# mlee03/FRE-NCtools

Measured on AMD Instinct MI355X. Metric: exchange-cells/s, higher is better.
Workload: dtype f64; 1 GPU; C384 cubed sphere (6 tiles) -> 1440x720 lat-lon, conservative_order2: exchange-grid search + centroid pass + CSR build per step; nxgrid=4160000, parallelism=1 latitude band(s) of the target, one per GPU, world_size=1

## Files before the change

### fre-nctools_amd/conserve_interp.py

```python
import ctypes as C
from dataclasses import dataclass, field
from typing import List, Optional

import numpy as np

from . import _lib
from ._lib import lib, check

CONSERVE_ORDER1 = 1
CONSERVE_ORDER2 = 2
TARGET = 16
READ = 256
WRITE = 512
CHECK_CONSERVE = 1024
LEGACY_CLIP = 2048
GREAT_CIRCLE = 4096
MONOTONIC = 16384
CELL_METHODS_MEAN = 0
CELL_METHODS_SUM = 1
MAXVAL = 1.0e20


def _f64(a):
    return np.ascontiguousarray(a, dtype=np.float64)
# ... 41 lines not shown


@dataclass
class FieldConfig:
    data: Optional[np.ndarray] = None
    grad_x: Optional[np.ndarray] = None
    grad_y: Optional[np.ndarray] = None
    grad_mask: Optional[np.ndarray] = None
    area: Optional[np.ndarray] = None
    var: List[VarConfig] = field(default_factory=lambda: [VarConfig()])


def _host_grid_args(grids_in, grid_out, masks):
    nt = len(grids_in)
    keep = []
    dpt = C.POINTER(C.c_double)

    def arr(a, n):
        a = _f64(a).reshape(-1)
        assert a.size == n, (a.size, n)
        keep.append(a)
        return _dp(a)

    def corners(g, a):
        return arr(a, (g.nx + 1) * (g.ny + 1))

    nx = (C.c_int * nt)(*[g.nx for g in grids_in])
    ny = (C.c_int * nt)(*[g.ny for g in grids_in])
    lon = (dpt * nt)(*[corners(g, g.lonc) for g in grids_in])
    lat = (dpt * nt)(*[corners(g, g.latc) for g in grids_in])
    msk = None
    if masks is not None:
        msk = (dpt * nt)(*[arr(m, g.nx * g.ny) if m is not None else dpt() for m, g in zip(masks, grids_in)])
    args = (nt, nx, ny, lon, lat, msk, grid_out.nx, grid_out.ny, corners(grid_out, grid_out.lonc), corners(grid_out, grid_out.latc))
    return args, keep


def _dev_grid_args(nx_in, ny_in, tables_t, masks_t, nx_out, ny_out, out_t, mean_dlat, mean_dlon, device, stream):
    nt = len(nx_in)
    tables = [(C.c_void_p * nt)(*[t.data_ptr() for t in tab]) for tab in tables_t]
    msk = None
    if masks_t is not None:
        msk = (C.c_void_p * nt)(*[(t.data_ptr() if t is not None else None) for t in masks_t])
    use = 0 if stream is None else 1
    sptr = C.c_void_p(0 if stream is None else int(stream))
    return (nt, (C.c_int * nt)(*nx_in), (C.c_int * nt)(*ny_in), *tables, msk, nx_out, ny_out, *[C.c_void_p(t.data_ptr()) for t in out_t],
            float(mean_dlat), float(mean_dlon), device, sptr, use)


class XgridPlan:

    def __init__(self, handle, order, device, great_circle=False):
        self._h = C.c_void_p(handle)
        self.order = order
        self.device = device
        self.great_circle = great_circle

    @classmethod
    def create(cls, order, grids_in, grid_out, masks=None, device=0):
        _lib.require_gpu()
        args, keep = _host_grid_args(grids_in, grid_out, masks)
        h = C.c_void_p()
        check(lib().fg_plan_create(order, *args, device, C.byref(h)))
        return cls(h.value, order, device)

    @classmethod
    def create_dev(cls, order, nx_in, ny_in, lon_in_t, lat_in_t, nx_out, ny_out, lon_out_t, lat_out_t,
                   mean_dlat=0.0, mean_dlon=0.0, device=0, stream=None, masks_t=None):
        h = C.c_void_p()
        check(lib().fg_plan_create_dev(order, *_dev_grid_args(nx_in, ny_in, (lon_in_t, lat_in_t), masks_t, nx_out, ny_out,
                                                              (lon_out_t, lat_out_t), mean_dlat, mean_dlon, device, stream), C.byref(h)))
        return cls(h.value, order, device)

    @classmethod
    def create_great_circle(cls, grids_in, grid_out, masks=None, device=0):
        _lib.require_gpu()
        args, keep = _host_grid_args(grids_in, grid_out, masks)
        h = C.c_void_p()
        check(lib().fg_plan_create_great_circle(*args, device, C.byref(h)))
        return cls(h.value, 1, device, True)

    @classmethod
    def create_great_circle_dev(cls, nx_in, ny_in, xyz_in_t, nx_out, ny_out, xyz_out_t, mean_dlat=0.0, mean_dlon=0.0,
                                device=0, stream=None, masks_t=None):
        h = C.c_void_p()
        tables = [[t[k] for t in xyz_in_t] for k in range(3)]
        check(lib().fg_plan_create_great_circle_dev(*_dev_grid_args(nx_in, ny_in, tables, masks_t, nx_out, ny_out, [xyz_out_t[k] for k in range(3)],
                                                                    mean_dlat, mean_dlon, device, stream), C.byref(h)))
        return cls(h.value, 1, device, True)

    @classmethod
    def create_great_circle_lonlat(cls, grids_in, grid_out, masks=None, device=0):
        _lib.require_gpu()
        args, keep = _host_grid_args(grids_in, grid_out, masks)
        h = C.c_void_p()
        check(lib().fg_plan_create_great_circle_lonlat(*args, device, C.byref(h)))
        return cls(h.value, 1, device, True)

    @classmethod
    def create_great_circle_lonlat_dev(cls, nx_in, ny_in, lon_in_t, lat_in_t, nx_out, ny_out, lon_out_t, lat_out_t,
                                       mean_dlat=0.0, mean_dlon=0.0, device=0, stream=None, masks_t=None):
        h = C.c_void_p()
        check(lib().fg_plan_create_great_circle_lonlat_dev(*_dev_grid_args(nx_in, ny_in, (lon_in_t, lat_in_t), masks_t, nx_out, ny_out,
                                                                           (lon_out_t, lat_out_t), mean_dlat, mean_dlon, device, stream),
                                                           C.byref(h)))
        return cls(h.value, 1, device, True)

    @classmethod
    def create_empty(cls, order, nx_in, ny_in, nx_out, ny_out, device=0):
        _lib.require_gpu()
        nt = len(nx_in)
        h = C.c_void_p()
        check(lib().fg_plan_create_empty(order, nt, (C.c_int * nt)(*nx_in), (C.c_int * nt)(*ny_in),
                                         nx_out, ny_out, device, C.byref(h)))
        return cls(h.value, order, device)

    def destroy(self):
        if self._h is not None and self._h.value:
            lib().fg_plan_destroy(self._h)
        self._h = None

    def __del__(self):
        try:
            self.destroy()
        except Exception:
            pass

    @property
    def nxgrid(self):
        return int(lib().fg_plan_nxgrid(self._h))

    @property
    def ncells_in(self):
        return int(lib().fg_plan_ncells_in(self._h))

    def cell_sums_ptr(self):
        return lib().fg_plan_cell_sums_dev(self._h)

    def copy_cell_sums(self, dst_t):
        check(lib().fg_plan_copy_cell_sums(self._h, C.c_void_p(dst_t.data_ptr())))

    def accumulate_cell_sums(self, total_t, cells_t=None):
        args = (self._h, C.c_void_p(total_t.data_ptr()), C.c_void_p(cells_t.data_ptr()) if cells_t is not None else None,
                int(cells_t.numel()) if cells_t is not None else 0)
        if getattr(total_t, "is_cuda", False):
            cur = _torch().cuda.current_stream(total_t.device)
            if int(self.stream() or 0) == int(cur.cuda_stream):
                check(lib().fg_plan_accumulate_cell_sums_async(*args))
                return
            cur.synchronize()
        check(lib().fg_plan_accumulate_cell_sums(*args))

    def stats(self):
        s = (C.c_long * 10)()
        check(lib().fg_plan_stats(self._h, s, 10))
        names = ["pairs", "nonempty", "nxgrid", "borderline", "bins", "bin_entries", "deferred", "heavy", "below", "exact_mode"]
        return dict(zip(names, [int(v) for v in s]))

    PHASES = ["cell_struct", "bins", "candidates", "clip_quad", "clip_general", "compact", "rows",
              "search_total", "finalize", "apply"]

    def phase_ms(self):
        ms = (C.c_float * 10)()
        check(lib().fg_plan_phase_ms(self._h, ms, 10))
        return dict(zip(self.PHASES, [float(v) for v in ms]))

    def finalize(self, total_sums_ptr=None):
        check(lib().fg_plan_finalize(self._h, C.c_void_p(total_sums_ptr or 0)))

    def sync(self):
        check(lib().fg_plan_sync(self._h))

    def stream(self):
        return lib().fg_plan_stream(self._h)

    def set_stream(self, stream):
        check(lib().fg_plan_set_stream(self._h, C.c_void_p(int(stream))))

    def get_xgrid(self):
        n = self.nxgrid
        ints = {k: np.empty(n, dtype=np.int32) for k in ("t_in", "i_in", "j_in", "i_out", "j_out")}
        area = np.empty(n, dtype=np.float64)
        c1 = np.empty(n, dtype=np.float64) if self.order == 2 else None
        c2 = np.empty(n, dtype=np.float64) if self.order == 2 else None
        check(lib().fg_plan_get_xgrid(self._h, _ip(ints["t_in"]), _ip(ints["i_in"]), _ip(ints["j_in"]),
                                      _ip(ints["i_out"]), _ip(ints["j_out"]), _dp(area), _dp(c1), _dp(c2)))
        out = dict(ints)
        out["area"] = area
        if self.order == 2:
            out["c1"], out["c2"] = c1, c2
        return out

    def get_polygons(self, maxv=16):
        nx = self.nxgrid
        n = np.zeros(nx, dtype=np.int32)
        v = [np.zeros((nx, maxv)) for _ in range(3)]
        check(lib().fg_plan_get_polygons(self._h, maxv, _ip(n), _dp(v[0]), _dp(v[1]), _dp(v[2])))
        if self.great_circle:
            return {"n": n, "x": v[0], "y": v[1], "z": v[2]}
        return {"n": n, "lon": v[0], "lat": v[1]}

    @classmethod
    def create_polylist(cls, order, n, lon, lat, lon_avg, area_ref, grid_out, device=0):
        _lib.require_gpu()
        n = np.ascontiguousarray(n, dtype=np.int32)
        lon, lat = _f64(lon), _f64(lat)
        assert lon.shape == (n.size, 8) == lat.shape
        lon_avg, area_ref = _f64(lon_avg), _f64(area_ref)
        lo, la = _f64(grid_out.lonc).reshape(-1), _f64(grid_out.latc).reshape(-1)
        h = C.c_void_p()
        check(lib().fg_plan_create_polylist(order, n.size, _ip(n), _dp(lon), _dp(lat), _dp(lon_avg), _dp(area_ref), grid_out.nx, grid_out.ny,
                                            _dp(lo), _dp(la), device, C.byref(h)))
        return cls(h.value, order, device)

    def get_cell_area(self, ncells_out):
        a_in = np.empty(self.ncells_in, dtype=np.float64)
        a_out = np.empty(ncells_out, dtype=np.float64)
        check(lib().fg_plan_get_cell_area(self._h, _dp(a_in), _dp(a_out)))
        return a_in, a_out

    def get_cell_struct(self, which, ncells):
        d = {k: np.empty(ncells, dtype=np.float64) for k in ("lat_min", "lat_max", "lon_min", "lon_max", "lon_avg")}
        nv = np.empty(ncells, dtype=np.int32)
        vlon = np.empty((ncells, 8), dtype=np.float64)
        vlat = np.empty((ncells, 8), dtype=np.float64)
        check(lib().fg_plan_get_cell_struct(self._h, which, _dp(d["lat_min"]), _dp(d["lat_max"]), _dp(d["lon_min"]),
                                            _dp(d["lon_max"]), _dp(d["lon_avg"]), _ip(nv), _dp(vlon), _dp(vlat)))
        d.update(nvert=nv, vlon=vlon, vlat=vlat)
        return d

    def set_xgrid(self, t_in, i_in, j_in, i_out, j_out, area, di_in=None, dj_in=None):
        a = [np.ascontiguousarray(v, dtype=np.int32) for v in (t_in, i_in, j_in, i_out, j_out)]
        area = _f64(area)
        di = _f64(di_in) if di_in is not None else None
        dj = _f64(dj_in) if dj_in is not None else None
        check(lib().fg_plan_set_xgrid(self._h, area.size, *[_ip(v) for v in a], _dp(area), _dp(di), _dp(dj)))

    def apply(self, data_t, out_t, nz=1, grad_x_t=None, grad_y_t=None, grad_mask_t=None,
              has_missing=False, missing=-MAXVAL, want_gsum=False):
        g = C.c_double(0.0)
        ptr = lambda t: C.c_void_p(t.data_ptr()) if t is not None else C.c_void_p(0)
        check(lib().fg_plan_apply(self._h, ptr(data_t), ptr(grad_x_t), ptr(grad_y_t), ptr(grad_mask_t),
                                  1 if has_missing else 0, float(missing), nz, ptr(out_t),
                                  C.byref(g) if want_gsum else None))
        return g.value if want_gsum else None


    def apply_ex(self, data_t, out_t, nz=1, grad_x_t=None, grad_y_t=None, grad_mask_t=None, has_missing=False,
                 missing=-MAXVAL, weight_t=None, cell_methods_sum=False, field_area_t=None, area_missing=-MAXVAL,
                 cell_area_in_t=None, cell_area_out_t=None, monotonic=False, want_gsum=False, minmax_hook=None):
        ptr = lambda t: C.c_void_p(t.data_ptr()) if t is not None else C.c_void_p(0)
        addr = lambda t: t.data_ptr() if t is not None else None
        o = _lib.ApplyOpts(1 if has_missing else 0, float(missing), addr(weight_t), 1 if cell_methods_sum else 0,
                           addr(field_area_t), float(area_missing), addr(cell_area_in_t), addr(cell_area_out_t),
                           1 if monotonic else 0)
        g = C.c_double(0.0)
        gp = C.byref(g) if want_gsum else None
        L = lib()
        if monotonic and self.order == 2 and minmax_hook is not None:
            check(L.fg_plan_mono_begin(self._h, C.byref(o), ptr(data_t), ptr(grad_x_t), ptr(grad_y_t), ptr(grad_mask_t)))
            minmax_hook(self)
            check(L.fg_plan_mono_end(self._h, C.byref(o), ptr(data_t), ptr(out_t), gp))
        else:
            check(L.fg_plan_apply_ex(self._h, C.byref(o), ptr(data_t), ptr(grad_x_t), ptr(grad_y_t), ptr(grad_mask_t),
                                     nz, ptr(out_t), gp))
        return g.value if want_gsum else None

    def mono_copy_minmax(self, to_plan, fmin_t, fmax_t):
        check(lib().fg_plan_mono_copy_minmax(self._h, 1 if to_plan else 0, C.c_void_p(fmin_t.data_ptr()),
                                              C.c_void_p(fmax_t.data_ptr())))

    def apply_interleaved(self, nb, data_il_t, out_il_t, grad_x_il_t=None, grad_y_il_t=None, want_gsum=False):
        g = C.c_double(0.0)
        ptr = lambda t: C.c_void_p(t.data_ptr()) if t is not None else C.c_void_p(0)
        check(lib().fg_plan_apply_interleaved(self._h, nb, ptr(data_il_t), ptr(grad_x_il_t), ptr(grad_y_il_t),
                                              ptr(out_il_t), C.byref(g) if want_gsum else None))
        return g.value if want_gsum else None

    def apply_records(self, nz, rec_t, out_t, want_gsum=False):
        g = C.c_double(0.0)
        check(lib().fg_plan_apply_records(self._h, nz, C.c_void_p(rec_t.data_ptr()), C.c_void_p(out_t.data_ptr()),
                                          C.byref(g) if want_gsum else None))
        return g.value if want_gsum else None

    def apply_levels(self, data_t, out_t, nlev, missing, grad_x_t=None, grad_y_t=None, grad_mask_t=None, want_gsum=False):
        g = np.zeros(nlev, dtype=np.float64)
        ptr = lambda t: C.c_void_p(t.data_ptr()) if t is not None else C.c_void_p(0)
        check(lib().fg_plan_apply_levels(self._h, ptr(data_t), ptr(grad_x_t), ptr(grad_y_t), ptr(grad_mask_t), float(missing),
                                         nlev, ptr(out_t), _dp(g) if want_gsum else None))
        return g if want_gsum else None

    def apply_records_levels(self, nz, rec_t, maskbits_t, out_t, missing, want_gsum=False):
        g = np.zeros(nz, dtype=np.float64)
        check(lib().fg_plan_apply_records_levels(self._h, nz, C.c_void_p(rec_t.data_ptr()), C.c_void_p(maskbits_t.data_ptr()),
                                                 float(missing), C.c_void_p(out_t.data_ptr()), _dp(g) if want_gsum else None))
        return g if want_gsum else None

    @staticmethod
    def levels_capacity():
        return int(lib().fg_plan_levels_capacity())


@dataclass
class InterpConfig:
    nxgrid: int = 0
    i_in: Optional[np.ndarray] = None
    j_in: Optional[np.ndarray] = None
    i_out: Optional[np.ndarray] = None
    j_out: Optional[np.ndarray] = None
# ... 248 lines not shown
```

### fre-nctools_amd/csrc/plan.hip

```cpp
#include <hip/hip_runtime.h>
#include <math.h>
#include <stdio.h>
#include <stdlib.h>
#include <string.h>
#include <algorithm>
#include <map>
#include <mutex>
#include <string>
#include <type_traits>
#include <vector>
#include "fg_host.h"
#include "xgrid_device.h"

static thread_local std::string g_err;
extern "C" const char *fg_last_error(void) { return g_err.c_str(); }
void fg_set_last_error(const char *msg) { g_err = msg ? msg : ""; }

extern "C" int fg_device_count(void)
{
  int n = 0;
  hipError_t e = hipGetDeviceCount(&n);
  if (e != hipSuccess) { fg_fail(FG_ERR_HIP, "hipGetDeviceCount: %s", hipGetErrorString(e)); return FG_ERR_HIP; }
  return n;
}
// ... 441 lines not shown
{
  static thread_local FgCounters *h = nullptr;
  if (!h) { if (hipHostMalloc((void **)&h, sizeof(FgCounters), hipHostMallocDefault) != hipSuccess) h = nullptr; }
  return h;
}

struct GcXyz { const double *x, *y, *z; };
struct BoxMode { FgBox box; const double *mask_quad; int no_adjust; };
struct SearchIn {
  const double *const *lon_in = nullptr, *const *lat_in = nullptr, *const *mask_in = nullptr;
  const double *lon_out = nullptr, *lat_out = nullptr;
  const GcXyz *gc_in = nullptr, *gc_out = nullptr;
  const BoxMode *boxm = nullptr;
  double mean_dlat = 0, mean_dlon = 0;
  int rect_hint = 1;
};
struct SearchOpts { bool exact, cull, finalize, rect, dst_frame; int gc_split; bool profile; };
static const char *gc_clip_error(int code)
{
  switch (code) {
    case 3: return "firstIntersect is not in the grid1List";
    case 4: return " not found the next intersection ";
    case 5: return "not return back to the first intersection";
    case 6: return "After clipping, nintersect should be 0";
    case 7: return "inserAfter: point (x,y,z) is not found in the list";
    case 8: return "Error from create_xgrid.c: temp is not in list1";
    default: return "clip_2dx2d_great_circle: more intersections than two convex quadrilaterals can have (list capacity)";
  }
}

static int g_search_cull = 0;
static int g_search_finalize = 0;
static int g_gc_split = 1;
extern "C" void fg_set_gc_split(int on) { g_gc_split = on < 0 ? 0 : on; }
struct SearchCaps { unsigned long long entries; int regcap, nreg; bool rect; };
static int g_search_rect = 1;
extern "C" void fg_set_search_rect(int on) { g_search_rect = on ? 1 : 0; }
static int g_dst_frame = 0;
extern "C" void fg_set_search_frame(int coupler) { g_dst_frame = coupler ? 1 : 0; }
static bool host_says_not_rect(int nx, int ny, const double *lon, const double *lat)
{
  const long nxp = nx + 1;
  const int js[3] = {ny, ny / 2, 1}, is[3] = {nx, nx / 2, 1};
  for (int a = 0; a < 3; a++)
    for (int b = 0; b < 3; b++) {
      const long e = (long)js[a] * nxp + is[b];
      if (memcmp(&lon[e], &lon[is[b]], sizeof(double)) || memcmp(&lat[e], &lat[(long)js[a] * nxp], sizeof(double))) return true;
    }
  return false;
}
#define FG_RETRY (-1000L)
struct Carve {
  size_t n = 0;
  size_t operator()(size_t size) { const size_t at = n; n += size; return at; }
};
struct SearchBlocks {
  fg_plan *pl;
  bool ok = true;
  std::vector<void *> scratch;
  template <typename T> T *keep(size_t count) { T *p = pl->alloc<T>(count); ok = ok && p; return p; }
  template <typename T> T *get(size_t count) { T *p = keep<T>(count); if (p) scratch.push_back(p); return p; }
  void release() { for (void *p : scratch) pl->release(p); scratch.clear(); }
};
static long plan_search_core(fg_plan *pl, const SearchIn &in, const SearchOpts &opt, SearchCaps *caps)
{
  const bool gc = in.gc_in != nullptr;
  const BoxMode *const boxm = in.boxm;
  pl->great_circle = gc;
  hipStream_t st = pl->stream;
  const int nsrc = pl->nsrc, ndst = pl->ndst, order = pl->order;
  FgCounters *hc = pinned_counters();
  if (!hc) return fg_fail(FG_ERR_HIP, "hipHostMalloc failed");

  std::vector<FgTile> &th = pl->tiles_host;
  th.resize(pl->ntiles + 1);
  for (int m = 0; m < pl->ntiles; m++) th[m] = FgTile{gc ? nullptr : in.lon_in[m], gc ? nullptr : in.lat_in[m], pl->nx_in[m], pl->ny_in[m], pl->cell_off[m]};
  th[pl->ntiles] = FgTile{in.lon_out, in.lat_out, pl->nx_out, pl->ny_out, 0};
  pl->tiles_dev = pl->alloc<FgTile>(pl->ntiles + 1);
  if (!pl->tiles_dev) return fg_fail(FG_ERR_HIP, "out of device memory");
  FgTileSet ts; ts.n = 0;
  const bool by_value = !gc && pl->ntiles + 1 <= FG_TILESET_MAX;
  if (by_value) { ts.n = pl->ntiles + 1; for (int m = 0; m <= pl->ntiles; m++) ts.t[m] = th[m]; }
  else FGCHK(hipMemcpyAsync(pl->tiles_dev, th.data(), sizeof(FgTile) * th.size(), hipMemcpyHostToDevice, st));
  FgTileXyz *gct_dev = nullptr;
  std::vector<FgTileXyz> gct;
  if (gc) {
    gct.resize(pl->ntiles + 1);
    for (int m = 0; m < pl->ntiles; m++) gct[m] = FgTileXyz{in.gc_in[m].x, in.gc_in[m].y, in.gc_in[m].z, pl->nx_in[m], pl->ny_in[m], pl->cell_off[m]};
    gct[pl->ntiles] = FgTileXyz{in.gc_out->x, in.gc_out->y, in.gc_out->z, pl->nx_out, pl->ny_out, 0};
    gct_dev = pl->alloc<FgTileXyz>(pl->ntiles + 1);
    if (!gct_dev) return fg_fail(FG_ERR_HIP, "out of device memory");
    FGCHK(hipMemcpyAsync(gct_dev, gct.data(), sizeof(FgTileXyz) * gct.size(), hipMemcpyHostToDevice, st));
  }

  bool any_mask = false;
  if (in.mask_in) for (int m = 0; m < pl->ntiles; m++) if (in.mask_in[m]) any_mask = true;
  if (any_mask) {
    pl->mask_dev = pl->alloc<double>(nsrc);
    if (!pl->mask_dev) return fg_fail(FG_ERR_HIP, "out of device memory");
    std::vector<double> ones;
    for (int m = 0; m < pl->ntiles; m++) {
      size_t nc = (size_t)pl->nx_in[m] * pl->ny_in[m];
      if (in.mask_in[m]) FGCHK(hipMemcpyAsync(pl->mask_dev + pl->cell_off[m], in.mask_in[m], nc * sizeof(double), hipMemcpyDeviceToDevice, st));
      else {
        ones.assign(nc, 1.0);
        FGCHK(hipMemcpyAsync(pl->mask_dev + pl->cell_off[m], ones.data(), nc * sizeof(double), hipMemcpyHostToDevice, st));
        FGCHK(hipStreamSynchronize(st));
      }
    }
  }

  const bool rect = caps->rect && !gc && !boxm;
  pl->rect = rect;
  const double dst_tlon = opt.dst_frame ? (double)NAN : 3.14159265358979323846;
  FgBins bins;
  choose_bins(pl, in.mean_dlat, in.mean_dlon, &bins);
  if (rect) { bins.nblat = 0; bins.nblon = 0; }
  const long nbins = (long)bins.nblat * bins.nblon;
  const long nslots = nbins + bins.nblat;
  const unsigned long long nentries = rect ? 0ull : caps->entries;
  const int ecap = (int)std::min<unsigned long long>(nentries, 2147483647ull);
  FgPairSpace ps{};
  ps.nreg = caps->nreg; ps.regcap = caps->regcap;
  const long npairs = fgd_pairs_total(ps);
  const long nx_alloc = npairs;

  if (!alloc_cells(pl, &pl->S, nsrc)) return fg_fail(FG_ERR_HIP, "out of device memory");
  SearchBlocks blk{pl};
  struct { double *hdr, *lat_ax, *lon_ax, *col, *row, *col_min, *col_max, *col_avg; } rt{};
  if (rect) {
    pl->D = FgCells{};
    pl->D.area = blk.keep<double>(ndst);
    Carve at;
    const size_t o_hdr = at(8), o_lat = at((size_t)pl->ny_out + 1), o_lon = at((size_t)pl->nx_out + 1), o_col = at(8 * (size_t)pl->nx_out),
                 o_row = at(4 * ((size_t)pl->ny_out + 1)), o_cmin = at((size_t)pl->nx_out), o_cmax = at((size_t)pl->nx_out), o_cavg = at((size_t)pl->nx_out);
    double *rect_blk = blk.keep<double>(at.n);
    if (!blk.ok) return fg_fail(FG_ERR_HIP, "out of device memory");
    rt = {rect_blk + o_hdr, rect_blk + o_lat, rect_blk + o_lon, rect_blk + o_col, rect_blk + o_row, rect_blk + o_cmin, rect_blk + o_cmax, rect_blk + o_cavg};
  } else if (!alloc_cells(pl, &pl->D, ndst)) return fg_fail(FG_ERR_HIP, "out of device memory");
  const long t_bins = fgd_scan_tiles(nslots), t_rows = fgd_scan_tiles(ndst), t_comp = fgd_scan_tiles(nsrc);
  const size_t zreg = (size_t)FG_NREG * FG_FILL_STRIDE * sizeof(unsigned);
  Carve z;
  const size_t z_dc = z((sizeof(FgCounters) + 127) / 128 * 128), z_fill = z(zreg), z_tick = z(128);
  const size_t z_lb_bins = z(t_bins * sizeof(unsigned long long)), z_lb_rows = z(t_rows * sizeof(unsigned long long)),
               z_lb_comp = z(t_comp * sizeof(unsigned long long));
  const size_t z_bin_cnt = z((size_t)(nslots + 1) * sizeof(int)), z_bin_fill = z((size_t)(nslots + 1) * sizeof(int)),
               z_row_cnt = z((size_t)(ndst + 1) * sizeof(int)), z_nacc = z((size_t)(nsrc + 1) * sizeof(int));
  z((16 - (z.n - z_bin_cnt) % 16) % 16);
  const size_t z_gc_ntask = z(gc ? zreg : 0), z_gc_ocnt = z(gc ? zreg : 0);
  const size_t zbytes = z.n;
  char *zero_blk = blk.get<char>(zbytes);
  int *bin_start = blk.get<int>(nslots + 1);
  int *heavy_list = blk.get<int>(nsrc + 1);
  int *big_list = blk.get<int>(nsrc + 1);
  int *pair_beg = blk.get<int>(nsrc + 1), *pair_cnt = blk.get<int>(nsrc + 1);
  FgBinEntry *bin_entries = blk.get<FgBinEntry>(nentries ? nentries : 1);
  ps.src = blk.get<int>(npairs + 1); ps.dst = blk.get<int>(npairs + 1);
  double *tmp_area = blk.get<double>(npairs + 1);
  double *tmp_clon = (order == 2) ? blk.get<double>(npairs + 1) : nullptr;
  double *tmp_clat = (order == 2) ? blk.get<double>(npairs + 1) : nullptr;
  int *defer_list = blk.get<int>(npairs + 1);
  const bool early_rows = !gc && !boxm;
  int *tmp_rowpos = early_rows ? blk.get<int>(npairs + 1) : nullptr;
  const bool gc_split = gc && opt.gc_split && npairs < (1L << 28);
  const long tcap_want = (opt.gc_split == 2) ? npairs / 64 : 3 * npairs;
  const long tcap_reg = gc_split ? std::min<long>((tcap_want / FG_NREG + 255) / 256 * 256, 0x7ffffff0L / FG_NREG) : 0;
  const long tcap_all = tcap_reg * FG_NREG;
  unsigned *gc_meta = gc_split ? blk.get<unsigned>(npairs + 1) : nullptr;
  int *gc_tbase = gc_split ? blk.get<int>(npairs + 1) : nullptr;
  int *gc_order = gc_split ? blk.get<int>(npairs + 1) : nullptr;
  unsigned *gc_task = gc_split ? blk.get<unsigned>(tcap_all + 1) : nullptr;
  double *gc_res = gc_split ? blk.get<double>(2 * (size_t)tcap_all + 2) : nullptr;
  pl->xoff = blk.keep<int>(nsrc + 1);
  pl->x_src = blk.keep<int>(nx_alloc + 1); pl->x_dst = blk.keep<int>(nx_alloc + 1);
  pl->x_area = blk.keep<double>(nx_alloc + 1);
  if (order == 2) { pl->x_c1 = blk.keep<double>(nx_alloc + 1); pl->x_c2 = blk.keep<double>(nx_alloc + 1); pl->sums = blk.keep<double>(3 * (size_t)nsrc); }
  int *x_rowpos = blk.get<int>(nx_alloc + 1);
  pl->perm = blk.keep<FgRowEnt>(nx_alloc + 1);
  pl->csr.row_ptr = blk.keep<int>(ndst + 1);
  if (!pl->src_idx_f) pl->src_idx_f = blk.keep<int>(nsrc + 1);
  if (!blk.ok) return fg_fail(FG_ERR_HIP, "out of device memory");
  FgCounters *dc = (FgCounters *)(zero_blk + z_dc);
  ps.fill = (unsigned *)(zero_blk + z_fill);
  unsigned *tickets = (unsigned *)(zero_blk + z_tick);
  unsigned long long *lb_bins = (unsigned long long *)(zero_blk + z_lb_bins), *lb_rows = (unsigned long long *)(zero_blk + z_lb_rows),
                     *lb_comp = (unsigned long long *)(zero_blk + z_lb_comp);
  int *bin_cnt = (int *)(zero_blk + z_bin_cnt), *bin_fill = (int *)(zero_blk + z_bin_fill), *row_cnt = (int *)(zero_blk + z_row_cnt);
  int *nacc = (int *)(zero_blk + z_nacc);
  FGCHK(hipMemsetAsync(zero_blk, 0, zbytes, st));
  if (pl->ll_err) FGCHK(hipMemcpyAsync(&dc->err[2], pl->ll_err, sizeof(unsigned), hipMemcpyDeviceToDevice, st));

  PhaseTimer pt, ptot;
  pt.start(opt.profile, st); ptot.start(opt.profile, st);
  for (int k = 0; k < PH_COUNT; k++) pl->phase_ms[k] = 0;
  ptot.begin(PH_SEARCH_TOTAL);
  pt.begin(PH_CELL_STRUCT);
  if (gc) {
    fgd_gc_cell_struct(gct_dev + pl->ntiles, 1, ndst, pl->D, st, opt.cull ? dc->band_keys : nullptr, 1);
    fgd_gc_cell_struct(gct_dev, pl->ntiles, nsrc, pl->S, st, opt.cull ? dc->band_keys : nullptr, 2);
    fgd_src_field_index(order, pl->tiles_dev, pl->ntiles, nsrc, pl->src_idx_f, st);
  } else if (rect) {
    FgRect &R = pl->rect_tab;
    R.hdr = rt.hdr; R.lat_ax = rt.lat_ax; R.lon_ax = rt.lon_ax; R.col = rt.col; R.row = rt.row;
    R.col_min = rt.col_min; R.col_max = rt.col_max; R.col_avg = rt.col_avg;
    R.bad = &dc->rect_bad; R.nx = pl->nx_out; R.ny = pl->ny_out;
    fgd_rect_tables(in.lon_out, in.lat_out, pl->nx_out, pl->ny_out, rt.hdr, rt.lat_ax, rt.lon_ax, rt.col, rt.col_min, rt.col_max, rt.col_avg, rt.row,
                    &dc->rect_bad, dc->err, st, dst_tlon);
    if (pl->polys.npoly) fgd_polylist_records(pl->polys, pl->S, pl->src_idx_f, pl->sums, &R, heavy_list, &dc->heavy_cnt, dc->err, st);
    fgd_cell_struct2r(ts, pl->tiles_dev, pl->tiles_dev, pl->ntiles, pl->polys.npoly ? 0 : nsrc, ndst, pl->S, pl->D.area, R, pl->mask_dev, order,
                      pl->src_idx_f, pl->sums, dc->err, st, dc->band_keys, (opt.cull && !pl->polys.npoly) ? 2 : 0, heavy_list, &dc->heavy_cnt,
                      ps, pair_beg, pair_cnt, big_list, &dc->big_cnt);
  } else if (opt.cull && !boxm && !pl->polys.npoly) {
    fgd_band_keys(in.lat_out, (long)(pl->nx_out + 1) * (pl->ny_out + 1), dc->band_keys, st);
    fgd_cell_struct2(ts, pl->tiles_dev, pl->tiles_dev, pl->ntiles, nsrc, ndst, pl->S, pl->D, bins, bin_cnt, order, pl->src_idx_f, pl->sums, dc->err, st, dc->band_keys, 2, dst_tlon);
  } else if (pl->polys.npoly) {
    fgd_polylist_records(pl->polys, pl->S, pl->src_idx_f, pl->sums, nullptr, nullptr, nullptr, dc->err, st);
    fgd_cell_struct2(ts, pl->tiles_dev, pl->tiles_dev, pl->ntiles, 0, ndst, pl->S, pl->D, bins, bin_cnt, order, pl->src_idx_f, pl->sums, dc->err, st, nullptr, 0, dst_tlon);
  } else
    fgd_cell_struct2(ts, pl->tiles_dev, pl->tiles_dev, pl->ntiles, nsrc, ndst, pl->S, pl->D, bins, bin_cnt, order, pl->src_idx_f, pl->sums, dc->err, st, nullptr, 0, dst_tlon);
  if (boxm) fgd_box_cell_boxes(boxm->box, pl->S, st);
  if (boxm && boxm->no_adjust) fgd_box_area_no_adjust(boxm->box, pl->S.area, st);
  pt.end();
  pl->have_geom = true;

  if (!rect) {
    pt.begin(PH_BINS);
    if (gc) fgd_bin_count(ndst, pl->D, bins, bin_cnt, st);
    fgd_exclusive_scan1(bin_cnt, nslots, bin_start, lb_bins, &tickets[0], &dc->total[0], dc->err, st);
    fgd_bin_fill(ndst, pl->D, bins, bin_fill, bin_start, bin_entries, ecap, nsrc, pl->S, pl->mask_dev, heavy_list, &dc->heavy_cnt, st);
    pt.end();
  }

  pt.begin(PH_CANDIDATES);
  if (rect)
    fgd_candidates_rect(nsrc, pl->S, pl->mask_dev, pl->rect_tab, ps, pair_beg, pair_cnt, heavy_list, &dc->heavy_cnt, big_list, &dc->big_cnt, st,
                        pl->polys.npoly ? 0 : 1);
  else
    fgd_candidates1(nsrc, pl->S, pl->mask_dev, bins, bin_start, bin_entries, ecap, ps, pair_beg, pair_cnt, heavy_list, &dc->heavy_cnt, big_list,
                    &dc->big_cnt, st);
  pt.end();
  hipEvent_t gc_e1 = nullptr, gc_e2 = nullptr;
  struct EvReturn {
    hipEvent_t &a, &b;
    ~EvReturn() { g_handles.put_sync_event(a); g_handles.put_sync_event(b); a = b = nullptr; }
  } ev_return{gc_e1, gc_e2};
  if (boxm) {
    pt.begin(PH_CLIP_GENERAL);
    fgd_clip_box(order, ps, boxm->box, th[pl->ntiles], pl->S, pl->D, pl->mask_dev, boxm->mask_quad, tmp_area, tmp_clon, tmp_clat, nacc, dc->stats, dc->err, st);
    pt.end();
  } else if (gc) {
    pt.begin(PH_CLIP_GENERAL);
    if (gc_split) {
      if (!pl->stream_b) pl->stream_b = g_handles.get_stream(pl->device);
      gc_e1 = g_handles.get_sync_event(); gc_e2 = g_handles.get_sync_event();
      GcSplit g{gc_meta, gc_tbase, gc_task, gc_res, (unsigned)tcap_reg, (unsigned *)(zero_blk + z_gc_ntask), defer_list, &dc->defer_cnt,
                &dc->gc_list2_cnt, npairs, gc_order, (unsigned *)(zero_blk + z_gc_ocnt)};
      fgd_gc_clip_split(ps, pl->S, pl->mask_dev, pl->D, tmp_area, nacc, g, dc->stats, dc->err, st, pl->stream_b, gc_e1, gc_e2);
    } else
      fgd_gc_clip(ps, pl->S, pl->mask_dev, pl->D, tmp_area, nacc, defer_list, &dc->defer_cnt, dc->stats, dc->err, st);
    pt.end();
  } else {
    pt.begin(PH_CLIP_QUAD);
    fgd_clip_quad(order, ps, pl->S, pl->mask_dev, pl->D, tmp_area, tmp_clon, tmp_clat, nacc, defer_list, &dc->defer_cnt, dc->stats, dc->err, st,
                  rect ? &pl->rect_tab : nullptr, row_cnt, tmp_rowpos);
    pt.end();
    pt.begin(PH_CLIP_GENERAL);
    fgd_clip_general(order, ps, pl->S, pl->mask_dev, pl->D, tmp_area, tmp_clon, tmp_clat, nacc, defer_list, &dc->defer_cnt, dc->stats, dc->err, st,
                     rect ? &pl->rect_tab : nullptr, row_cnt, tmp_rowpos);
    pt.end();
  }
  pt.begin(PH_COMPACT);
  FgCompactIo io{};
  io.pair_beg = pair_beg; io.pair_cnt = pair_cnt;
  io.tmp_area = tmp_area; io.tmp_clon = tmp_clon; io.tmp_clat = tmp_clat;
  io.xoff = pl->xoff; io.x_src = pl->x_src; io.x_dst = pl->x_dst; io.x_area = pl->x_area; io.x_c1 = pl->x_c1; io.x_c2 = pl->x_c2;
  io.row_cnt = row_cnt; io.x_rowpos = x_rowpos; io.sums = pl->sums; io.big_list = big_list; io.big_cnt = &dc->big_cnt;
  io.tmp_rowpos = tmp_rowpos; io.row_ptr = pl->csr.row_ptr; io.perm = pl->perm;
  io.dc = dc; io.xcap = nx_alloc;
  if (early_rows)
    fgd_exclusive_scan2(nacc, nsrc, pl->xoff, lb_comp, &tickets[2], &dc->xtot, row_cnt, ndst, pl->csr.row_ptr, lb_rows, &tickets[1], &dc->rows_total, dc->err, st);
  else
    fgd_exclusive_scan1(nacc, nsrc, pl->xoff, lb_comp, &tickets[2], &dc->xtot, dc->err, st);
  fgd_compact(order, nsrc, ps, io, st);
  pt.end();
  if (!early_rows) {
    pt.begin(PH_ROWS);
    fgd_exclusive_scan1(row_cnt, ndst, pl->csr.row_ptr, lb_rows, &tickets[1], &dc->rows_total, dc->err, st);
    fgd_csr_fill_pos(nx_alloc, &dc->xtot, pl->x_src, pl->x_dst, pl->csr.row_ptr, x_rowpos, pl->perm, st);
    pt.end();
  }
  ptot.end();
  const bool fuse = opt.finalize && early_rows && !pl->polys.npoly;
  int *fused_tmp = nullptr;
  if (fuse) {
    pt.begin(PH_FINALIZE);
    if (order == 2) {
      pl->cen = pl->alloc<FgSrcRec>((size_t)nsrc + 1);
      if (!pl->cen) return fg_fail(FG_ERR_HIP, "out of device memory");
      fgd_centroids(nsrc, pl->S, pl->sums, pl->cen, st);
      pl->csr.e2 = pl->alloc<FgCsrEntry2>(nx_alloc + 1);
    } else pl->csr.e1 = pl->alloc<FgCsrEntry1>(nx_alloc + 1);
    if (!pl->csr.e1 && !pl->csr.e2) return fg_fail(FG_ERR_HIP, "out of device memory");
    int *sg_tmp = pl->alloc<int>(3 * (size_t)(nx_alloc + 1));
    fgd_csr_sortgather(order, ndst, (long)nsrc + ndst, pl->perm, pl->x_area, pl->x_c1, pl->x_c2, pl->src_idx_f,
                       order == 2 ? pl->cen : nullptr, pl->csr, st, sg_tmp, nx_alloc + 1);
    fused_tmp = sg_tmp;
    pt.end();
  }
  FGCHK(hipMemcpyAsync(hc, dc, sizeof(FgCounters), hipMemcpyDeviceToHost, st));
  FGCHK(hipStreamSynchronize(st));
  pt.collect(pl->phase_ms); ptot.collect(pl->phase_ms);
  FGCHK(hipGetLastError());
  if (rect && hc->rect_bad) { caps->rect = false; return FG_RETRY; }
  if (hc->total[0] > nentries) { caps->entries = hc->total[0]; return FG_RETRY; }
  if (hc->total[0] > 2000000000ull) return fg_fail(FG_ERR_ARG, "bin table too large");
  if (hc->total[3] > (unsigned long long)ps.regcap) {
    if (hc->total[3] > 2000000000ull / (unsigned long long)ps.nreg) return fg_fail(FG_ERR_CAPACITY, "candidate pair list exceeds 2^31 entries");
    caps->regcap = (int)((hc->total[3] + FG_REG_ALIGN - 1) / FG_REG_ALIGN * FG_REG_ALIGN);
    return FG_RETRY;
  }
  if (hc->err[2] & G_ERRBIT_LL2X) return fg_fail(FG_ERR_ARG, "latlon2xyz: a grid corner is not finite, or its latitude (|lat| >= 2.4262) or longitude "
                                                          "(|lon| > 1024) lies outside the range of the device trig (radians expected)");
  if (hc->err[0] & 8u) return fg_fail(FG_ERR_ARG, "a grid corner latitude lies outside [-pi/2, pi/2] (radians expected)");
  if (hc->err[0] & 1u) return fg_fail(FG_ERR_MAXV, "create_xgrid.c: n2_in is greater than MAX_V");
  if (hc->err[0] & 2u) return fg_fail(FG_ERR_PARALLEL, "the line between <x1_0,y1_0> and  <x1_1,y1_1> should not parallel to "
                                                    "the line between <x2_0,y2_0> and  <x2_1,y2_1>");
  if (hc->err[0] & 4u) return fg_fail(FG_ERR_MAXV, "clipped polygon exceeds 16 vertices");
  if (hc->err[0] & G_ERRBIT_GC_CONVEX1) return fg_fail(FG_ERR_GEOM, "create_xgrid.c(clip_2dx2d_great_circle): grid box 1 is not convex");
  if (hc->err[0] & G_ERRBIT_GC_CONVEX2) return fg_fail(FG_ERR_GEOM, "create_xgrid.c(clip_2dx2d_great_circle): grid box 2 is not convex");
  if (hc->err[0] & G_ERRBIT_GC_CLIP) return fg_fail(FG_ERR_GEOM, "%s", gc_clip_error((int)hc->err[1]));
  if (hc->err[0] & G_ERRBIT_LOOKBACK) return fg_fail(FG_ERR_HIP, "single-pass scan: a tile waited too long for its predecessor");
  pl->nx = (long)hc->xtot;
  pl->stats[FG_STAT_PAIRS] = (long)hc->total[1];
  pl->stats[FG_STAT_NONEMPTY] = (long)(hc->xtot + hc->stats[FG_STAT_BELOW]);
  pl->stats[FG_STAT_NXGRID] = pl->nx;
  pl->stats[FG_STAT_BORDERLINE] = (long)hc->stats[FG_STAT_BORDERLINE];
  pl->stats[FG_STAT_BINS] = nbins;
  pl->stats[FG_STAT_BIN_ENTRIES] = (long)hc->total[0];
  pl->stats[FG_STAT_DEFERRED] = hc->defer_cnt + hc->gc_list2_cnt;
  pl->stats[FG_STAT_HEAVY] = hc->heavy_cnt;
  pl->stats[FG_STAT_BELOW] = (long)hc->stats[FG_STAT_BELOW];

  pl->rect_tab.bad = nullptr;
  blk.release();
  pl->rows_built = true;
  pl->searched = true;
  if (fuse) {
    pl->release(pl->perm); pl->perm = nullptr; pl->release(fused_tmp);
    if (!pl->red_partial) { pl->red_partial = pl->alloc<double>(1024); pl->red_result = pl->alloc<double>(260); }
    if (!pl->red_partial || !pl->red_result) return fg_fail(FG_ERR_HIP, "out of device memory");
    pl->dist_pending = (order == 2);
    pl->finalized = true; pl->fused = true;
  }
  return pl->nx;
}

static int g_search_exact = 0;
extern "C" void fg_set_search_mode(int exact) { g_search_exact = exact; }
extern "C" void fg_set_search_cull(int on) { g_search_cull = on ? 1 : 0; }
extern "C" void fg_set_search_finalize(int on) { g_search_finalize = on ? 1 : 0; }
static long plan_search(fg_plan *pl, const SearchIn &in)
{
  static const bool env_exact = getenv("FREGRID_HIP_EXACT_SEARCH") && atoi(getenv("FREGRID_HIP_EXACT_SEARCH")) != 0;
  const SearchOpts opt{.exact = g_search_exact || env_exact, .cull = g_search_cull != 0, .finalize = g_search_finalize != 0,
                       .rect = g_search_rect != 0, .dst_frame = g_dst_frame != 0, .gc_split = g_gc_split, .profile = g_profiling != 0};
  const long big = std::max((long)pl->nsrc, (long)pl->ndst);
  if (big > (1L << 28)) return fg_fail(FG_ERR_CAPACITY, "grid of %ld cells: more than 2^28 cells per search are not supported", big);
  SearchCaps caps;
  caps.entries = opt.exact ? 0ull : 3ull * (unsigned long long)pl->ndst + 4096ull;
  const unsigned long long cap_pairs = std::min<unsigned long long>(8ull * (unsigned long long)big + 65536ull, 2000000000ull);
  caps.nreg = (int)std::max(1L, std::min((long)FG_NREG, ((long)pl->nsrc + 1023) / 1024));
  caps.regcap = opt.exact ? 0 : (int)((cap_pairs / caps.nreg + FG_REG_ALIGN - 1) / FG_REG_ALIGN * FG_REG_ALIGN);
  caps.rect = opt.rect && in.rect_hint && !in.gc_in && !in.boxm && pl->nx_out <= 8192 && pl->nx_out >= 2;
  const size_t keep = pl->owned.size();
  long rc = FG_RETRY;
  int attempts = 0;
  for (; attempts < 4 && rc == FG_RETRY; attempts++) {
    if (attempts) {
      (void)hipStreamSynchronize(pl->stream);
      pl->drop_search(keep);
    }
    rc = plan_search_core(pl, in, opt, &caps);
  }
  if (rc == FG_RETRY) return fg_fail(FG_ERR_CAPACITY, "exchange-grid search: capacities did not settle");
  if (rc >= 0) pl->stats[FG_STAT_EXACT] = (attempts > 1) ? 1 : 0;
  return rc;
}

struct CornerSample {
  int nsamp = 0;
  std::vector<double> q;
  const double *corners(int a, int k) const { return &q[((size_t)a * nsamp + k) * 4]; }
};
static long sample_step(int nx, int ny, int *nsamp)
{
  const long ncell = (long)nx * ny;
  long step = ncell / 4096; if (step < 1) step = 1;
  *nsamp = (int)((ncell + step - 1) / step);
  return step;
}
__host__ __device__ static inline void sample_nodes(int nx, long step, int k, long n[4])
{
  const long c = (long)k * step;
  const int i = (int)(c % nx), j = (int)(c / nx);
  n[0] = (long)j * (nx + 1) + i; n[1] = n[0] + 1; n[3] = n[0] + nx + 1; n[2] = n[3] + 1;
}
static CornerSample sample_corners_host(int nx, int ny, int narr, const double *const *arr)
{
  CornerSample s;
  const long step = sample_step(nx, ny, &s.nsamp);
  s.q.resize((size_t)s.nsamp * narr * 4);
  for (int k = 0; k < s.nsamp; k++) {
    long n[4];
    sample_nodes(nx, step, k, n);
    for (int a = 0; a < narr; a++)
      for (int v = 0; v < 4; v++) s.q[((size_t)a * s.nsamp + k) * 4 + v] = arr[a][n[v]];
  }
  return s;
}
__global__ void k_sample_corners(int nx, long step, int nsamp, int narr, const double *a0, const double *a1, const double *a2, double *out)
{
  const int k = blockIdx.x * blockDim.x + threadIdx.x;
  if (k >= nsamp) return;
  long n[4];
  sample_nodes(nx, step, k, n);
  const double *arr[3] = {a0, a1, a2};
  for (int a = 0; a < narr; a++) {
    double *o = out + ((size_t)a * nsamp + k) * 4;
    o[0] = arr[a][n[0]]; o[1] = arr[a][n[1]]; o[2] = arr[a][n[2]]; o[3] = arr[a][n[3]];
  }
}
static int sample_corners_dev(fg_plan *pl, int nx, int ny, int narr, const double *d_a0, const double *d_a1, const double *d_a2, CornerSample *s)
{
  const long step = sample_step(nx, ny, &s->nsamp);
  s->q.resize((size_t)s->nsamp * narr * 4);
  double *d_q = (double *)g_pool.get(pl->device, s->q.size() * sizeof(double));
  if (!d_q) return fg_fail(FG_ERR_HIP, "out of device memory");
  k_sample_corners<<<(s->nsamp + 255) / 256, 256, 0, pl->stream>>>(nx, step, s->nsamp, narr, d_a0, d_a1, d_a2, d_q);
  hipError_t e = hipMemcpyAsync(s->q.data(), d_q, s->q.size() * sizeof(double), hipMemcpyDeviceToHost, pl->stream);
  if (e == hipSuccess) e = hipStreamSynchronize(pl->stream);
  g_pool.put(d_q);
  if (e != hipSuccess) return fg_fail(FG_ERR_HIP, "sampling the destination corners failed: %s", hipGetErrorString(e));
  return 0;
}
static void mean_extents(double sl, double sw, long cnt, double *mdlat, double *mdlon)
{
  const double PI = 3.14159265358979323846;
  if (cnt == 0) { *mdlat = PI / 180; *mdlon = PI / 180; return; }
  *mdlat = sl / cnt; *mdlon = sw / cnt;
  if (*mdlat < 1e-7) *mdlat = 1e-7;
  if (*mdlon < 1e-7) *mdlon = 1e-7;
}
static void extents_lonlat(const CornerSample &s, double *mdlat, double *mdlon, int *curvilinear)
{
  const double PI = 3.14159265358979323846;
  *curvilinear = 0;
  double sl = 0, sw = 0; long cnt = 0;
  for (int k = 0; k < s.nsamp; k++) {
    const double *x = s.corners(0, k), *y = s.corners(1, k);
    if (memcmp(&x[0], &x[3], 8) || memcmp(&x[1], &x[2], 8) || memcmp(&y[0], &y[1], 8) || memcmp(&y[3], &y[2], 8)) *curvilinear = 1;
    double ymin = y[0], ymax = y[0], w = 0;
    for (int m = 1; m < 4; m++) { if (y[m] < ymin) ymin = y[m]; if (y[m] > ymax) ymax = y[m]; }
    for (int m = 0; m < 4; m++) {
      double d = fabs(x[(m + 1) & 3] - x[m]);
      if (d > 3.0 * PI) d = fabs(remainder(d, 2.0 * PI)); else if (d > PI) d = fabs(2.0 * PI - d);
      if (d > w) w = d;
    }
    if (w > PI / 2) continue;
    sl += ymax - ymin; sw += w; cnt++;
  }
  mean_extents(sl, sw, cnt, mdlat, mdlon);
}
static void extents_xyz(const CornerSample &s, double *mdlat, double *mdlon)
{
  double sl = 0, sw = 0; long cnt = 0;
  for (int k = 0; k < s.nsamp; k++) {
    const double *x = s.corners(0, k), *y = s.corners(1, k), *z = s.corners(2, k);
    const double dx = x[0] - x[2], dy = y[0] - y[2], dz = z[0] - z[2];
    const double diag = sqrt(dx * dx + dy * dy + dz * dz);
    const double zc = 0.5 * (z[0] + z[2]);
    const double coslat = sqrt(fmax(0.0, 1.0 - zc * zc));
    if (coslat < 0.2) continue;
    sl += diag; sw += diag / coslat; cnt++;
  }
  mean_extents(sl, sw, cnt, mdlat, mdlon);
}
struct DstExtents { double dlat = 0, dlon = 0; int rect_hint = 1; };
static DstExtents dst_extents_host(int nx, int ny, const double *lon, const double *lat)
{
  const double *arr[2] = {lon, lat};
  DstExtents x;
  int curvilinear;
  extents_lonlat(sample_corners_host(nx, ny, 2, arr), &x.dlat, &x.dlon, &curvilinear);
// ... 1695 lines not shown
```

### fre-nctools_amd/csrc/xgrid_device.h

```cpp
#pragma once
#include <hip/hip_runtime.h>

struct FgTile {
  const double *lon;
  const double *lat;
  int nx, ny;
  int cell_off;
};

struct FgTileXyz {
  const double *x, *y, *z;
  int nx, ny;
  int cell_off;
};
#define G_ERRBIT_GC_CONVEX1 16u
#define G_ERRBIT_GC_CONVEX2 32u
#define G_ERRBIT_GC_CLIP    64u

struct FgCells {
  double *lat_min, *lat_max, *lon_min, *lon_max, *lon_avg, *area;
  int *nv;
  double *verts;
};

struct FgBins {
  int nblat, nblon;
  double inv_wlat, inv_wlon;
};

struct FgBinEntry {
  double lat_min, lat_max, lon_min, lon_max, lon_avg;
  int d;
  int row0;
};

enum {
  FG_STAT_PAIRS = 0,
  FG_STAT_NONEMPTY = 1,
  FG_STAT_NXGRID = 2,
  FG_STAT_BORDERLINE = 3,
  FG_STAT_BINS = 4,
  FG_STAT_BIN_ENTRIES = 5,
  FG_STAT_DEFERRED = 6,
  FG_STAT_HEAVY = 7,
  FG_STAT_BELOW = 8,
  FG_STAT_EXACT = 9,
  FG_NSTATS = 10
};

#define FG_REG_ALIGN 512
#define FG_NREG 64
#define FG_FILL_STRIDE 32
struct FgPairSpace {
  int *src, *dst;
  unsigned *fill;
  int regcap, nreg;
};
#ifdef __HIPCC__
__device__ __forceinline__ bool d_pair_live(const FgPairSpace &ps, int p)
{
  const unsigned first = blockIdx.x * blockDim.x;
  const unsigned r = first / (unsigned)ps.regcap;
  const unsigned f = ps.fill[r * FG_FILL_STRIDE];
  return (unsigned)p - r * (unsigned)ps.regcap < (f < (unsigned)ps.regcap ? f : (unsigned)ps.regcap);
}
#endif
static inline long fgd_pairs_total(const FgPairSpace &ps) { return (long)ps.regcap * ps.nreg; }
#ifdef __HIPCC__
__device__ __forceinline__ unsigned long long d_ord_key(double v)
{
  const unsigned long long b = (unsigned long long)__double_as_longlong(v);
  return (b >> 63) ? ~b : (b | 0x8000000000000000ull);
}
__device__ __forceinline__ double d_ord_val(unsigned long long k)
{
  const unsigned long long b = (k >> 63) ? (k & 0x7fffffffffffffffull) : ~k;
  return __longlong_as_double((long long)b);
}
#endif

#define FG_TILESET_MAX 8
struct FgTileSet { FgTile t[FG_TILESET_MAX]; int n; };

struct FgLl2xGrid { const double *lon, *lat; double *x, *y, *z; long n; };
struct FgLl2xSet { FgLl2xGrid g[FG_TILESET_MAX]; int n; };
#define G_ERRBIT_LL2X 256u
void fgd_latlon2xyz(const FgLl2xGrid *grids, int ngrids, unsigned *err, hipStream_t st);

struct FgCounters {
  unsigned long long total[4];
  unsigned long long rows_total;
  unsigned long long band_keys[2];
  unsigned long long xtot;
  unsigned err[4];
  int heavy_cnt;
  unsigned rect_bad;
  int defer_cnt, big_cnt;
  int gc_list2_cnt;
  unsigned long long stats[FG_NSTATS];
};
#define G_ERRBIT_LOOKBACK 128u

long fgd_scan_tiles(long n);
void fgd_exclusive_scan1(const int *in, long n, int *out, unsigned long long *status, unsigned *ticket,
                         unsigned long long *total_dev, unsigned *err, hipStream_t st);

void fgd_exclusive_scan2(const int *in_a, long n_a, int *out_a, unsigned long long *status_a, unsigned *ticket_a, unsigned long long *total_a,
                         const int *in_b, long n_b, int *out_b, unsigned long long *status_b, unsigned *ticket_b, unsigned long long *total_b,
                         unsigned *err, hipStream_t st);

void fgd_cell_struct2(const FgTileSet &ts, const FgTile *tiles_in, FgTile *tiles_out, int ntiles, int nsrc, int ndst, FgCells S, FgCells D,
                      FgBins b, int *slot_cnt, int order, int *src_idx_f, double *sums, unsigned *err, hipStream_t st,
                      unsigned long long *band_keys = nullptr, int cull = 0, double dst_tlon = 3.14159265358979323846);
void fgd_cell_struct(const FgTile *tiles_dev, int ntiles, int ncells, FgCells c, unsigned *err, hipStream_t st);
void fgd_band_keys(const double *lat, long n, unsigned long long *band_keys, hipStream_t st);
void fgd_bin_count(int ncells, FgCells c, FgBins b, int *slot_cnt, hipStream_t st);
void fgd_bin_fill(int ndst, FgCells D, FgBins b, int *slot_fill, const int *slot_start, FgBinEntry *entries, int cap,
                  int nsrc, FgCells S, const double *mask, int *heavy_list, int *heavy_cnt, hipStream_t st);
void fgd_candidates1(int nsrc, FgCells S, const double *mask, FgBins b, const int *slot_start, const FgBinEntry *entries, int ecap,
                     FgPairSpace ps, int *pair_beg, int *pair_cnt, const int *heavy_list, const int *heavy_cnt, int *big_list, int *big_cnt,
                     hipStream_t st);
#define RECT_COLW 8
struct FgRect {
  const double *lon_ax;
  const double *lat_ax;
  const double *col;
  const double *col_min, *col_max, *col_avg;
  const double *hdr;
  const double *row;
  const unsigned *bad;
  int nx, ny;
};
void fgd_rect_tables(const double *lon, const double *lat, int nx, int ny, double *hdr, double *lat_ax, double *lon_ax, double *col,
                     double *col_min, double *col_max, double *col_avg, double *row, unsigned *bad, unsigned *err, hipStream_t st,
                     double dst_tlon = 3.14159265358979323846);
void fgd_cell_struct2r(const FgTileSet &ts, const FgTile *tiles_in, FgTile *tiles_out, int ntiles, int nsrc, int ndst, FgCells S, double *area_out,
                       FgRect R, const double *mask, int order, int *src_idx_f, double *sums, unsigned *err, hipStream_t st,
                       unsigned long long *band_keys, int cull, int *heavy_list, int *heavy_cnt, FgPairSpace ps, int *pair_beg, int *pair_cnt,
                       int *big_list, int *big_cnt);
void fgd_rect_materialize(int ndst, FgRect R, FgCells D, hipStream_t st);
struct FgPolyList { const int *n; const double *lon, *lat; const double *lon_avg, *area; int npoly; };
void fgd_polylist_records(FgPolyList P, FgCells S, int *src_idx_f, double *sums, const FgRect *rect, int *heavy_list, int *heavy_cnt,
                          unsigned *err, hipStream_t st);
void fgd_candidates_rect(int nsrc, FgCells S, const double *mask, FgRect R, FgPairSpace ps, int *pair_beg, int *pair_cnt,
                         const int *heavy_list, const int *heavy_cnt, int *big_list, int *big_cnt, hipStream_t st, int listed_only);
void fgd_clip_general(int order, FgPairSpace ps, FgCells S, const double *mask, FgCells D,
              double *tmp_area, double *tmp_clon, double *tmp_clat, int *nacc, int *defer_list, int *defer_cnt,
              unsigned long long *stats, unsigned *err, hipStream_t st, const FgRect *rect = nullptr, int *row_cnt = nullptr,
              int *tmp_rowpos = nullptr);
void fgd_clip_quad(int order, FgPairSpace ps, FgCells S, const double *mask, FgCells D,
              double *tmp_area, double *tmp_clon, double *tmp_clat, int *nacc, int *defer_list, int *defer_cnt,
              unsigned long long *stats, unsigned *err, hipStream_t st, const FgRect *rect = nullptr, int *row_cnt = nullptr,
              int *tmp_rowpos = nullptr);
struct alignas(8) FgRowEnt { int n, s; };
struct alignas(16) FgSrcRec { double cen_lon, cen_lat; };
struct FgCompactIo {
  const int *pair_beg, *pair_cnt;
  const double *tmp_area, *tmp_clon, *tmp_clat;
  const int *xoff;
  int *x_src, *x_dst;
  double *x_area, *x_c1, *x_c2;
  int *row_cnt, *x_rowpos;
  const int *tmp_rowpos;
  const int *row_ptr; FgRowEnt *perm;
  double *sums;
  const int *big_list;
  const int *big_cnt;
  FgCounters *dc;
  long xcap;
};
void fgd_compact(int order, int nsrc, FgPairSpace ps, const FgCompactIo &io, hipStream_t st);
void fgd_centroids(int nsrc, FgCells S, const double *sums, FgSrcRec *cen, hipStream_t st);
void fgd_distances(long nx, const int *x_src, const double *x_area, const FgSrcRec *cen, double *x_c1, double *x_c2, hipStream_t st);

struct FgCsrEntry1 { int idx_f; int pad; double area; };
struct FgCsrEntry2 { int idx_f; int idx_g; double area, di, dj; };
struct FgCsr {
  int *row_ptr;
  FgCsrEntry1 *e1;
  FgCsrEntry2 *e2;
};
void fgd_csr_count(long nx, const int *x_dst, int *row_cnt, hipStream_t st);
void fgd_csr_fill(long nx, const int *x_src, const int *x_dst, const int *row_ptr, int *row_fill, FgRowEnt *perm, hipStream_t st);
void fgd_csr_fill_pos(long nx_cap, const unsigned long long *nx_dev, const int *x_src, const int *x_dst, const int *row_ptr, const int *x_rowpos,
                      FgRowEnt *perm, hipStream_t st);
void fgd_csr_sortgather(int order, int ndst, long nx, const FgRowEnt *perm, const double *x_area, const double *x_c1, const double *x_c2,
                        const int *src_idx_f, const FgSrcRec *cen, FgCsr csr, hipStream_t st, int *tmp = nullptr, long ntmp = 0,
                        int long_rows = 0);
void fgd_src_field_index(int order, const FgTile *tiles_dev, int ntiles, int nsrc, int *src_idx_f, hipStream_t st);
void fgd_apply1(int order, int ndst, FgCsr csr, const double *f, const double *gx, const double *gy, const int *gmask,
                int has_missing, double missing, double *out, double *row_sum, hipStream_t st, long nx = -1);
void fgd_apply_il(int order, int nb, int ndst, FgCsr csr, const double *f, const double *gx, const double *gy, double missing,
                  double *out, double *row_sum, long out_ld, int nb_valid, hipStream_t st, long nx = -1);
void fgd_interleave(int nb_pad, long n, const double *in, long ld, int nb_valid, double *out, hipStream_t st);
void fgd_apply_il_merged(int nb, int ndst, long nx, FgCsr csr, const double *rec, double missing, double *out, double *row_sum, long out_ld,
                         int nb_valid, hipStream_t st);
void fgd_merge3(int nb_pad, long n, const int *src_idx_f, const double *f, long ld_f, const double *gx, const double *gy, long ld_g,
                int nb_valid, double *out, hipStream_t st);
void fgd_interleave3(int nb_pad, int narr, const double *const *in, const long *ld, const long *n, double *const *out, int nb_valid,
                     hipStream_t st);
void fgd_deinterleave(int nb_pad, long n, const double *in, long ld, int nb_valid, double *out, hipStream_t st);
#define FG_LEVELS_CAP 256
void fgd_apply_levels8(int order, int ndst, long nx, FgCsr csr, const double *rec, const unsigned char *gbits, double missing, double *out,
                       double *row_sum, long ld, int nb_valid, hipStream_t st);
void fgd_gmask_bits(long n, const int *gmask, long ld, int nb, unsigned char *bits, hipStream_t st);
void fgd_apply_frac(int ndst, FgCsr csr, const double *data, double *out, hipStream_t st);
void fgd_reduce_sum(const double *v, long n, double *partial, double *result, hipStream_t st);
void fgd_xgrid_indices(long nx, const int *x_src, const int *x_dst, const FgTile *tiles_dev, int ntiles, int nx_out,
                       int *t_in, int *i_in, int *j_in, int *i_out, int *j_out, hipStream_t st);

struct FgApplyEx {
  const double *weight;
  const double *cell_area;
  const double *field_area;
  const double *cell_area_out;
  const int *gmask;
  const double *xdata;
  double area_missing, missing;
  int has_missing, sum;
};
#define FG_XERR_AREA_MISSING 1
#define FG_XERR_ABOVE 2
#define FG_XERR_BELOW 4
void fgd_apply_ex(int order, int ndst, FgCsr csr, const double *f, const double *gx, const double *gy, FgApplyEx o,
                  double *out, double *row_sum, int *err, hipStream_t st, long nx = -1);
void fgd_mono_bounds(const FgTile *tiles_dev, int ntiles, int nsrc, const int *src_idx_f, const double *f, double missing,
                     double *fbmax, double *fbmin, double *fmax, double *fmin, hipStream_t st);
void fgd_mono_xdata(long nx, FgCsr csr, const double *f, const double *gx, const double *gy, const int *gmask, double missing,
                    double *xdata, double *fmax, double *fmin, hipStream_t st);
void fgd_mono_limit(long nx, FgCsr csr, const double *f, double missing, const double *fbmax, const double *fbmin,
                    const double *fmax, const double *fmin, double *xdata, int *err, hipStream_t st);

struct FgBox { const double *lon, *lat; int nx, ny; };
void fgd_clip_box(int order, FgPairSpace ps, FgBox box, FgTile quad, FgCells S, FgCells D,
                  const double *mask_box, const double *mask_quad, double *tmp_area, double *tmp_clon, double *tmp_clat, int *nacc,
                  unsigned long long *stats, unsigned *err, hipStream_t st);
void fgd_box_area_no_adjust(FgBox box, double *area, hipStream_t st);
void fgd_box_cell_boxes(FgBox box, FgCells c, hipStream_t st);
void fgd_clip_single(const double *lon_in, const double *lat_in, int n_in, double ll_lon, double ll_lat, double ur_lon, double ur_lat,
                     double *lon_out, double *lat_out, int *n_out, hipStream_t st);
void fgd_box_ctr(double ll_lon, double ll_lat, double ur_lon, double ur_lat, double clon, double *out, hipStream_t st);
void fgd_grid_area_no_adjust(int nx, int ny, const double *lon, const double *lat, double *area, hipStream_t st);

void fgd_accumulate_cell_sums(int n, const int *cells, int nsrc, const int *xoff, const double *xa, const double *c1, const double *c2,
                              double *total, hipStream_t st);

void fgd_gc_cell_struct(const FgTileXyz *tiles_dev, int ntiles, int ncells, FgCells c, hipStream_t st,
                        unsigned long long *band_keys = nullptr, int band_mode = 0);
void fgd_gc_clip(FgPairSpace ps, FgCells S, const double *mask, FgCells D,
                 double *tmp_area, int *nacc, int *defer_list, int *defer_cnt, unsigned long long *stats, unsigned *err, hipStream_t st);
struct GcSplit {
  unsigned *meta;
  int *tbase;
  unsigned *task;
  double *res;
  unsigned tcap;
  unsigned *ntask;
  int *list, *list_cnt;
  int *list2_cnt;
  long list_cap;
  int *order;
  unsigned *ocnt;
};
void fgd_gc_clip_split(FgPairSpace ps, FgCells S, const double *mask, FgCells D, double *tmp_area, int *nacc, GcSplit g,
                       unsigned long long *stats, unsigned *err, hipStream_t st, hipStream_t st2, hipEvent_t e1, hipEvent_t e2);
#define FG_GC_POLY_CAP 16
void fgd_gc_clip_batch(int n, const double *a, const double *b, double *out, int *n_out, double *area, hipStream_t st);
void fgd_gc_area_batch(int npoly, int stride_pts, const double *xyz, const int *n, double *area, hipStream_t st);

#define FG_POLY_STRIDE 24
void fgd_poly_clip(int npoly, const double *lon1, const double *lat1, const int *n1, const double *lon2, const double *lat2,
                   const int *n2, double *lon_out, double *lat_out, int *n_out, hipStream_t st);
void fgd_poly_op(int op, int npoly, double *lon, double *lat, int *n, const double *clon, double *result, hipStream_t st);
void fgd_xgrid_polygons(long n, const int *x_src, const int *x_dst, FgCells S, FgCells D, const FgRect *rect, int maxv,
                        int *n_out, double *lon_out, double *lat_out, hipStream_t st);
void fgd_xgrid_gather_gc(long n, const int *x_src, const int *x_dst, FgCells S, FgCells D, double *a, double *b, hipStream_t st);
void fgd_split_xyz(long n, int maxv, const double *xyz, double *x, double *y, double *z, hipStream_t st);
void fgd_sincos_probe(long n, const double *x, double *s, double *c, hipStream_t st);

void fgd_pack_interior(const void *tiles, int ntiles, long ncells, long F, int nz, const double *src, double *dst, hipStream_t st);
void fgd_halo_gather(long F, int nz, const int *map, double *data, hipStream_t st);
void fgd_grad_c2l(const void *tiles, int ntiles, long ncells, long F, int nz, const double *data, const double *const *geom,
                  double *grad_x, double *grad_y, hipStream_t st);
void fgd_grad_c2l_rec(const void *tiles, int ntiles, long ncells, long F, int nz, int nb_pad, const double *data,
                      const double *const *geom, double *rec, hipStream_t st);
void fgd_c2l_records(const void *tiles, int ntiles, long ncells, int nz, int nb_pad, const double *src, const int *cell_of,
                     const double *const *geom, double *rec, hipStream_t st);
void fgd_c2l_records_levels(const void *tiles, int ntiles, long ncells, int nz, const double *src, const int *cell_of,
                            const double *const *geom, double missing, double *rec, unsigned char *gbits, hipStream_t st);
void fgd_grad_mask(const void *tiles, int ntiles, long ncells, long F, int nz, const double *data, double missing, int *mask, hipStream_t st);
size_t fgd_c2l_tile_size(void);
void fgd_c2l_tile_fill(void *dst, int idx, int nx, int ny, long cell_off, long f_off, long dx_off, long dy_off, long ew_off, long es_off);
```

### fre-nctools_amd/csrc/xgrid_kernels.hip

```cpp
#include <algorithm>
#include "xgrid_device.h"
#ifndef FG_EXP
#define FG_EXP 0
#endif
static __shared__ double fgs_lds_tab[112 * 4];
#define FGS_TAB(k, j) fgs_lds_tab[(k) * 4 + (j)]
#include "geom.hip.h"
__device__ __forceinline__ void d_load_trig_table()
{
  for (int i = threadIdx.x; i < 112 * 4; i += blockDim.x) fgs_lds_tab[i] = FG_SINCOS_TAB[i >> 2][i & 3];
  __syncthreads();
}

#define SCAN_THREADS 256
#define SCAN_ITEMS   8
#define SCAN_CHUNK   (SCAN_THREADS * SCAN_ITEMS)
#define LB_AGG   (1ull << 62)
#define LB_INC   (2ull << 62)
#define LB_MASK  ((1ull << 62) - 1ull)
#define LB_SPIN_LIMIT (1u << 22)

__device__ __forceinline__ unsigned wave_incl_scan(unsigned v, int lane)
{
#pragma unroll
// ... 15 lines not shown
#pragma unroll
  for (int k = 0; k < 4; k++) { if (k < w) base += wsum[k]; tot += wsum[k]; }
  __syncthreads();
  *total = tot;
  return inc + base;
}

__device__ __forceinline__ unsigned long long lb_load(const unsigned long long *p)
{
  return __hip_atomic_load(p, __ATOMIC_RELAXED, __HIP_MEMORY_SCOPE_AGENT);
}
__device__ __forceinline__ void lb_store(unsigned long long *p, unsigned long long v)
{
  __hip_atomic_store(p, v, __ATOMIC_RELAXED, __HIP_MEMORY_SCOPE_AGENT);
}

__device__ inline unsigned long long d_lookback_wave(unsigned long long *status, int tile, unsigned long long agg, unsigned *err)
{
  const int lane = threadIdx.x & 63;
  if (tile == 0) { if (lane == 0) lb_store(&status[0], LB_INC | (agg & LB_MASK)); return 0ull; }
  if (lane == 0) lb_store(&status[tile], LB_AGG | (agg & LB_MASK));
  unsigned long long excl = 0ull;
  int base = tile - 1;
  unsigned spins = 0;
  for (;;) {
    const int t = base - lane;
    const unsigned long long v = (t >= 0) ? lb_load(&status[t]) : LB_INC;
    const unsigned flag = (unsigned)(v >> 62);
    const unsigned long long inc = __ballot(flag == 2u), zero = __ballot(flag == 0u);
    const int first_inc = inc ? (__ffsll((long long)inc) - 1) : 63;
    const unsigned long long need = (first_inc >= 63) ? ~0ull : ((2ull << first_inc) - 1ull);
    if (zero & need) {
      if (++spins > LB_SPIN_LIMIT) { if (lane == 0) atomicOr(err, G_ERRBIT_LOOKBACK); break; }
      __builtin_amdgcn_s_sleep(1);
      continue;
    }
    unsigned long long val = ((need >> lane) & 1ull) ? (v & LB_MASK) : 0ull;
#pragma unroll
    for (int o = 32; o; o >>= 1) val += __shfl_xor(val, o);
    excl += val;
    if (inc) break;
    base -= 64;
  }
  if (lane == 0) lb_store(&status[tile], LB_INC | ((excl + agg) & LB_MASK));
  return excl;
}

__global__ __launch_bounds__(SCAN_THREADS) void k_scan1(const int *in, long n, int *out, unsigned long long *status, unsigned *ticket,
                                                        unsigned long long *total_out, unsigned *err)
{
  __shared__ unsigned tile[SCAN_CHUNK];
  __shared__ int sh_t;
  __shared__ unsigned long long sh_excl;
  if (ticket) { if (threadIdx.x == 0) sh_t = (int)atomicAdd(ticket, 1u); __syncthreads(); }
  const int t = ticket ? sh_t : (int)blockIdx.x;
  const long base = (long)t * SCAN_CHUNK;
#pragma unroll
  for (int k = 0; k < SCAN_ITEMS; k++) {
    const int li = k * SCAN_THREADS + threadIdx.x;
    const long idx = base + li;
    tile[li] = (idx < n) ? (unsigned)in[idx] : 0u;
  }
  __syncthreads();
  unsigned loc[SCAN_ITEMS];
  unsigned s = 0;
#pragma unroll
  for (int k = 0; k < SCAN_ITEMS; k++) { loc[k] = tile[threadIdx.x * SCAN_ITEMS + k]; s += loc[k]; }
  unsigned tot;
  const unsigned inc = block_incl_scan(s, &tot);
  if (threadIdx.x < 64) {
    const unsigned long long e = d_lookback_wave(status, t, (unsigned long long)tot, err);
    if (threadIdx.x == 0) sh_excl = e;
  }
  __syncthreads();
  const unsigned long long excl = sh_excl;
  unsigned run = (unsigned)excl + inc - s;
#pragma unroll
  for (int k = 0; k < SCAN_ITEMS; k++) { tile[threadIdx.x * SCAN_ITEMS + k] = run; run += loc[k]; }
  __syncthreads();
#pragma unroll
  for (int k = 0; k < SCAN_ITEMS; k++) {
    const int li = k * SCAN_THREADS + threadIdx.x;
    const long idx = base + li;
    if (idx <= n) out[idx] = (int)tile[li];
  }
  if (threadIdx.x == 0 && n >= base && n < base + SCAN_CHUNK) *total_out = excl + tot;
}

struct FgScanJob { const int *in; long n; int *out; unsigned long long *status; unsigned *ticket; unsigned long long *total; };
__global__ __launch_bounds__(SCAN_THREADS) void k_scan2(FgScanJob a, FgScanJob b, unsigned *err, int by_ticket)
{
  const FgScanJob j = blockIdx.y ? b : a;
  const long nt = (j.n + 1 + SCAN_CHUNK - 1) / SCAN_CHUNK;
  if ((long)blockIdx.x >= nt) return;
  __shared__ unsigned tile[SCAN_CHUNK];
  __shared__ int sh_t;
  __shared__ unsigned long long sh_excl;
  if (by_ticket) { if (threadIdx.x == 0) sh_t = (int)atomicAdd(j.ticket, 1u); __syncthreads(); }
  const int t = by_ticket ? sh_t : (int)blockIdx.x;
  const long base = (long)t * SCAN_CHUNK;
#pragma unroll
  for (int k = 0; k < SCAN_ITEMS; k++) {
    const int li = k * SCAN_THREADS + threadIdx.x;
    const long idx = base + li;
    tile[li] = (idx < j.n) ? (unsigned)j.in[idx] : 0u;
  }
  __syncthreads();
  unsigned loc[SCAN_ITEMS];
  unsigned s = 0;
#pragma unroll
  for (int k = 0; k < SCAN_ITEMS; k++) { loc[k] = tile[threadIdx.x * SCAN_ITEMS + k]; s += loc[k]; }
  unsigned tot;
  const unsigned inc = block_incl_scan(s, &tot);
  if (threadIdx.x < 64) {
    const unsigned long long e = d_lookback_wave(j.status, t, (unsigned long long)tot, err);
    if (threadIdx.x == 0) sh_excl = e;
  }
  __syncthreads();
  const unsigned long long excl = sh_excl;
  unsigned run = (unsigned)excl + inc - s;
#pragma unroll
  for (int k = 0; k < SCAN_ITEMS; k++) { tile[threadIdx.x * SCAN_ITEMS + k] = run; run += loc[k]; }
  __syncthreads();
#pragma unroll
  for (int k = 0; k < SCAN_ITEMS; k++) {
    const int li = k * SCAN_THREADS + threadIdx.x;
    const long idx = base + li;
    if (idx <= j.n) j.out[idx] = (int)tile[li];
  }
  if (threadIdx.x == 0 && j.n >= base && j.n < base + SCAN_CHUNK) *j.total = excl + tot;
}

long fgd_scan_tiles(long n) { if (n < 0) n = 0; return (n + 1 + SCAN_CHUNK - 1) / SCAN_CHUNK; }
void fgd_exclusive_scan2(const int *in_a, long n_a, int *out_a, unsigned long long *status_a, unsigned *ticket_a, unsigned long long *total_a,
                         const int *in_b, long n_b, int *out_b, unsigned long long *status_b, unsigned *ticket_b, unsigned long long *total_b,
                         unsigned *err, hipStream_t st)
{
  if (n_a < 0) n_a = 0;
  if (n_b < 0) n_b = 0;
  const long nt = std::max(fgd_scan_tiles(n_a), fgd_scan_tiles(n_b));
  k_scan2<<<dim3((unsigned)nt, 2), SCAN_THREADS, 0, st>>>(FgScanJob{in_a, n_a, out_a, status_a, ticket_a, total_a},
                                                         FgScanJob{in_b, n_b, out_b, status_b, ticket_b, total_b}, err, 2 * nt > 1024 ? 1 : 0);
}

void fgd_exclusive_scan1(const int *in, long n, int *out, unsigned long long *status, unsigned *ticket,
                         unsigned long long *total_dev, unsigned *err, hipStream_t st)
{
  if (n < 0) n = 0;
  const int nt = (int)fgd_scan_tiles(n);
  k_scan1<<<nt, SCAN_THREADS, 0, st>>>(in, n, out, status, nt <= 1024 ? nullptr : ticket, total_dev, err);
}


__device__ __forceinline__ int d_cell_record(const FgTile *tiles, int ntiles, int ncells, const FgCells &c, unsigned *err, int s0,
                                             double *vtile, double *box , int *tile_of,
                                             const unsigned long long *cull = nullptr, double tlon = G_PI)
{
  const int s = s0 + threadIdx.x;
  double *row = vtile + threadIdx.x * 17;
#pragma unroll
  for (int k = 0; k < 16; k++) row[k] = 0.0;
  int nvert = 0;
  if (s < ncells) {
    int t = 0;
    while (t + 1 < ntiles && s >= tiles[t + 1].cell_off) t++;
    *tile_of = t;
    const FgTile T = tiles[t];
    int loc = s - T.cell_off;
    int i = loc % T.nx, j = loc / T.nx;
    int nxp = T.nx + 1;
    int n0 = j * nxp + i, n1 = n0 + 1, n3 = n0 + nxp, n2 = n3 + 1;
    double x[G_FIXCAP], y[G_FIXCAP];
    x[0] = T.lon[n0]; y[0] = T.lat[n0];
    x[1] = T.lon[n1]; y[1] = T.lat[n1];
    x[2] = T.lon[n2]; y[2] = T.lat[n2];
    x[3] = T.lon[n3]; y[3] = T.lat[n3];
    double lmin = y[0], lmax = y[0];
#pragma unroll
    for (int k = 1; k < 4; k++) { if (y[k] < lmin) lmin = y[k]; if (y[k] > lmax) lmax = y[k]; }
    c.lat_min[s] = lmin; c.lat_max[s] = lmax;
    box[0] = lmin; box[1] = lmax;
    if (!(lmin >= -G_HPI - 1.e-6) || !(lmax <= G_HPI + 1.e-6)) atomicOr(err, G_ERRBIT_BADLAT);
    bool out_of_band = false;
    if (cull && cull[0]) {
      const double bmax = d_ord_val(cull[0]), bmin = d_ord_val(~cull[1]);
      out_of_band = (lmax <= bmin) || (lmin >= bmax);
    }
    int n = out_of_band ? 0 : d_fix_lon_quad_fast(x, y, tlon);
    if (n < 0) n = d_fix_lon(x, y, 4, tlon);
    if (out_of_band) { c.nv[s] = 0; c.area[s] = 0; }
    else if (n < 0 || n > G_MAXV) {
      atomicOr(err, G_ERRBIT_MAXV);
      c.nv[s] = 0; c.lon_min[s] = 0; c.lon_max[s] = 0; c.lon_avg[s] = 0; c.area[s] = 0;
    } else {
      double xmin = x[0], xmax = x[0], xs = 0;
      for (int k = 1; k < n; k++) { if (x[k] < xmin) xmin = x[k]; if (x[k] > xmax) xmax = x[k]; }
      for (int k = 0; k < n; k++) xs += x[k];
      xs /= n;
      c.lon_min[s] = xmin; c.lon_max[s] = xmax; c.lon_avg[s] = xs;
      box[2] = xmin; box[3] = xmax; box[4] = xs;
      c.nv[s] = n;
      nvert = n;
      for (int k = 0; k < G_MAXV; k++) {
        row[k] = (k < n) ? x[k] : 0.0;
        row[8 + k] = (k < n) ? y[k] : 0.0;
      }
      c.area[s] = d_poly_area<1>(x, y, n);
    }
  }
  if (!__syncthreads_or(nvert != 0) && cull) return 0;
  const long cnt = (long)min(256, ncells - s0) * 16;
  double *out = c.verts + (size_t)s0 * 16;
#pragma unroll
  for (int q = 0; q < 16; q++) {
    const long e = (long)q * 256 + threadIdx.x;
    if (e < cnt) out[e] = vtile[(e >> 4) * 17 + (e & 15)];
  }
  return nvert;
}

__global__ __launch_bounds__(256) void k_cell_struct(const FgTile *tiles, int ntiles, int ncells, FgCells c, unsigned *err)
{
  __shared__ double vtile[256 * 17];
  d_load_trig_table();
  double box[5]; int tl = 0;
  (void)d_cell_record(tiles, ntiles, ncells, c, err, blockIdx.x * 256, vtile, box, &tl);
}

__device__ __forceinline__ void d_cell_box(double lat_min, double lat_max, double lon_min, double lon_max, FgBins b,
                                           int *r0, int *r1, long long *l0, long long *l1)
{
  const double eps = 1.e-9;
  int a0 = (int)floor((lat_min - eps + G_HPI) * b.inv_wlat);
  int a1 = (int)floor((lat_max + eps + G_HPI) * b.inv_wlat);
  *r0 = max(0, min(b.nblat - 1, a0));
  *r1 = max(0, min(b.nblat - 1, a1));
  *l0 = (long long)floor((lon_min - eps) * b.inv_wlon);
  *l1 = (long long)floor((lon_max + eps) * b.inv_wlon);
}
__device__ __forceinline__ int d_colmod(long long l, int nb) { return (int)(((l % nb) + nb) % nb); }

__device__ __forceinline__ int d_slot_position(int *slot_cnt, int key)
{
  const int lane = threadIdx.x & 63;
  const int prev = __shfl_up(key, 1);
  const bool head = (lane == 0) || (key != prev);
  const unsigned long long heads = __ballot(head);
  const int start = 63 - __clzll((long long)(heads & ((2ull << lane) - 1ull)));
  const unsigned long long above = (start == 63) ? 0ull : (heads & ~((2ull << start) - 1ull));
  const int end = above ? (__ffsll((long long)above) - 1) : 64;
  int base = 0;
  if (lane == start && key >= 0) base = atomicAdd(&slot_cnt[key], end - start);
  base = __shfl(base, start);
  return base + (lane - start);
}

#define BIN_COPIES 16
#define BIN_ROW_COPIES 4
static_assert(BIN_COPIES >= 1 && BIN_COPIES <= 16, "a bin record keeps the copy number and copies - 1 in four bits each");

__device__ __forceinline__ bool d_copy_first(int word, int c_start, int nblon, bool first_row)
{
  const int col = word & 0xffff, o = (word >> 16) & 15, flen = ((word >> 20) & 15) + 1;
  if (((word >> 24) & 1) && !first_row) return false;
  int p = col - c_start;
  if (p < 0) p += nblon;
  return p == 0 || (o == 0 && p + flen <= nblon);
}

template <bool FILL>
__device__ __forceinline__ void d_bin_insert(bool live, int d, double lat_min, double lat_max, double lon_min, double lon_max, double lon_avg,
                                             FgBins b, int *slot_cnt, const int *slot_start, FgBinEntry *entries, int cap)
{
  FgBinEntry E;
  int r0 = 0, r1 = 0; long long l0 = 0, l1 = 0;
  if (live) {
    E.lat_min = lat_min; E.lat_max = lat_max; E.lon_min = lon_min; E.lon_max = lon_max; E.lon_avg = lon_avg;
    E.d = d;
    d_cell_box(lat_min, lat_max, lon_min, lon_max, b, &r0, &r1, &l0, &l1);
    E.row0 = r0;
  }
  const int nbins = b.nblat * b.nblon;
  const int maxcopies = (b.nblon <= 0xffff) ? min(BIN_COPIES, b.nblon) : 1, maxrows_c = (b.nblon <= 0xffff) ? BIN_ROW_COPIES : 1;
  const bool regular = live && r1 - r0 <= maxrows_c && l1 - l0 <= maxcopies;
  const int ccopies = regular ? max(1, (int)(l1 - l0)) : 0, rcopies = regular ? max(1, r1 - r0) : 0;
  const int ncopies = ccopies * rcopies;
  int maxc = ncopies;
#pragma unroll
  for (int o = 32; o; o >>= 1) maxc = max(maxc, __shfl_xor(maxc, o));
  for (int k = 0; k < maxc; k++) {
    const bool on = k < ncopies;
    const int kr = on ? k / ccopies : 0, kc = on ? k - kr * ccopies : 0;
    const int col = on ? d_colmod(l0 + kc, b.nblon) : 0;
    const int slot = on ? (r0 + kr) * b.nblon + col : -1;
    if (FILL) {
      const int pos = d_slot_position(slot_cnt, slot);
      if (on) {
        const int at = slot_start[slot] + pos;
        E.row0 = (col & 0xffff) | (kc << 16) | ((ccopies - 1) << 20) | ((kr > 0) << 24);
        if ((unsigned)at < (unsigned)cap) entries[at] = E;
      }
    } else if (on)
      atomicAdd(&slot_cnt[slot], 1);
  }
  E.row0 = r0;
  const int nrows = (live && !regular) ? (r1 - r0 + 1) : 0;
  int maxrows = nrows;
#pragma unroll
  for (int o = 32; o; o >>= 1) maxrows = max(maxrows, __shfl_xor(maxrows, o));
  for (int it = 0; it < maxrows; it++) {
    const int key = (it < nrows) ? nbins + r0 + it : -1;
    const int pos = d_slot_position(slot_cnt, key);
    if (FILL && key >= 0) { const int at = slot_start[key] + pos; if ((unsigned)at < (unsigned)cap) entries[at] = E; }
  }
}

__global__ __launch_bounds__(256) void k_cell_struct2(FgTileSet ts, const FgTile *tiles_in, FgTile *tiles_out, int ntiles, int nsrc, int ndst,
                                                       int nbS, FgCells S, FgCells D, FgBins b, int *slot_cnt, int order, int *src_idx_f,
                                                       double *sums, unsigned *err, unsigned long long *band_keys, int cull, double dst_tlon)
{
  __shared__ double vtile[256 * 17];
  __shared__ FgTile sh_tiles[FG_TILESET_MAX];
  if (ts.n && (int)threadIdx.x < ts.n) sh_tiles[threadIdx.x] = ts.t[threadIdx.x];
  const bool isD = (int)blockIdx.x >= nbS;
  if (cull && !isD && band_keys[0]) {
    __syncthreads();
    const FgTile *tl0 = ts.n ? sh_tiles : tiles_in;
    const int s = blockIdx.x * 256 + threadIdx.x;
    bool keep = false;
    int idx_f = s;
    if (s < nsrc) {
      int t = 0;
      while (t + 1 < ntiles && s >= tl0[t + 1].cell_off) t++;
      const int loc = s - tl0[t].cell_off, i = loc % tl0[t].nx, j = loc / tl0[t].nx, nxp = tl0[t].nx + 1;
      if (order == 2) {
        int foff = 0;
        for (int m = 0; m < t; m++) foff += (tl0[m].nx + 2) * (tl0[m].ny + 2);
        idx_f = foff + (j + 1) * (tl0[t].nx + 2) + i + 1;
      }
      const int n0 = j * nxp + i;
      const double y0 = tl0[t].lat[n0], y1 = tl0[t].lat[n0 + 1], y2 = tl0[t].lat[n0 + nxp + 1], y3 = tl0[t].lat[n0 + nxp];
      const double lmin = fmin(fmin(y0, y1), fmin(y2, y3)), lmax = fmax(fmax(y0, y1), fmax(y2, y3));
      const double bmax = d_ord_val(band_keys[0]), bmin = d_ord_val(~band_keys[1]);
      keep = !((lmax <= bmin) || (lmin >= bmax)) || !(lmin == lmin);
    }
    if (!__syncthreads_or(keep)) {
      if (s < nsrc) {
        S.nv[s] = 0; S.area[s] = 0;
        if (src_idx_f) src_idx_f[s] = idx_f;
        if (sums) { sums[s] = 0.0; sums[nsrc + s] = 0.0; sums[2 * (size_t)nsrc + s] = 0.0; }
      }
      if (ts.n && blockIdx.x == 0 && (int)threadIdx.x < ts.n) tiles_out[threadIdx.x] = sh_tiles[threadIdx.x];
      return;
    }
  }
  d_load_trig_table();
  const FgTile *tiles = ts.n ? sh_tiles : tiles_in;
  if (ts.n && blockIdx.x == 0 && (int)threadIdx.x < ts.n) tiles_out[threadIdx.x] = sh_tiles[threadIdx.x];
  double box[5] = {0, 0, 0, 0, 0};
  int tl = 0;
  if (!isD) {
    const int s0 = blockIdx.x * 256, s = s0 + threadIdx.x;
    (void)d_cell_record(tiles, ntiles, nsrc, S, err, s0, vtile, box, &tl, cull ? band_keys : nullptr);
    if (s < nsrc && sums) { sums[s] = 0.0; sums[nsrc + s] = 0.0; sums[2 * (size_t)nsrc + s] = 0.0; }
    if (s < nsrc && src_idx_f) {
      if (order != 2) src_idx_f[s] = s;
      else {
        int foff = 0;
        for (int t = 0; t < tl; t++) foff += (tiles[t].nx + 2) * (tiles[t].ny + 2);
        const int loc = s - tiles[tl].cell_off, i = loc % tiles[tl].nx, j = loc / tiles[tl].nx;
        src_idx_f[s] = foff + (j + 1) * (tiles[tl].nx + 2) + i + 1;
// ... 302 lines not shown
                                                      double *lon_ax, double *col, double *col_min, double *col_max, double *col_avg, double *row,
                                                      unsigned *bad, unsigned *err, double dst_tlon)
{
  d_load_trig_table();
  const long np = (long)(nx + 1) * (ny + 1);
  const long gid = (long)blockIdx.x * 256 + threadIdx.x, gsz = (long)gridDim.x * 256;
  bool b = false;
  for (long e = gid; e < np; e += gsz) {
    const long j = e / (nx + 1); const int i = (int)(e - j * (nx + 1));
    if (__double_as_longlong(lon[e]) != __double_as_longlong(lon[i]) ||
        __double_as_longlong(lat[e]) != __double_as_longlong(lat[j * (nx + 1)])) b = true;
  }
  if (gid <= ny) {
    const double y = lat[gid * (nx + 1)];
    lat_ax[gid] = y;
    if (!(y >= -G_HPI - 1.e-6) || !(y <= G_HPI + 1.e-6)) atomicOr(err, G_ERRBIT_BADLAT);
    if (gid < ny && !(lat[(gid + 1) * (nx + 1)] > y)) b = true;
    if (gid > 0 && gid < ny && d_is_pole(y)) b = true;
    double *r = row + (size_t)gid * 4;
    r[0] = d_sin_lat(0.5 * (y + y));
    if (gid < ny) {
      const double yb = lat[(gid + 1) * (nx + 1)];
      const bool flat = fabs(yb - y) < G_SMALL;
      const double dy = 0.5 * (yb - y);
      r[1] = d_sin_lat(0.5 * (yb + y)); r[2] = flat ? 1.0 : d_sin_lat(dy) / dy; r[3] = flat ? 1.0 : 0.0;
    } else { r[1] = 0.0; r[2] = 1.0; r[3] = 1.0; }
  }
  if (gid <= nx) lon_ax[gid] = lon[gid];
  if (gid < nx) {
    const double x0 = lon[gid], x1 = lon[gid + 1];
    if (!(x1 > x0) || !(x1 - x0 < G_PI - 1.e-6)) b = true;
    double x[G_FIXCAP], y[G_FIXCAP];
    x[0] = x0; x[1] = x1; x[2] = x1; x[3] = x0;
    y[0] = 0.0; y[1] = 0.0; y[2] = 0.1; y[3] = 0.1;
    const int n = d_fix_lon(x, y, 4, dst_tlon);
    double *c = col + (size_t)gid * RECT_COLW;
    if (n != 4) { b = true; for (int k = 0; k < RECT_COLW; k++) c[k] = 0.0; col_min[gid] = 0.0; col_max[gid] = 0.0; col_avg[gid] = 0.0; }
    else {
      double xmin = x[0], xmax = x[0], xs = 0;
      for (int k = 1; k < 4; k++) { if (x[k] < xmin) xmin = x[k]; if (x[k] > xmax) xmax = x[k]; }
      for (int k = 0; k < 4; k++) xs += x[k];
      xs /= 4;
      c[0] = x[0]; c[1] = x[1]; c[2] = x[2]; c[3] = x[3]; c[4] = xmin; c[5] = xmax; c[6] = xs; c[7] = x1 - x0;
      col_min[gid] = xmin; col_max[gid] = xmax; col_avg[gid] = xs;
    }
  }
  if (gid == 0) {
    if (!(lon[nx] - lon[0] <= G_TPI + 1.e-9)) b = true;
    hdr[0] = lon[0]; hdr[1] = nx / (lon[nx] - lon[0]); hdr[2] = lat[0]; hdr[3] = ny / (lat[(long)ny * (nx + 1)] - lat[0]);
  }
  if (__ballot(b) && (threadIdx.x & 63) == 0) atomicOr(bad, 1u);
}

template <bool STRICT>
__device__ __forceinline__ int d_axis_first(const double *ax, int n, double v, double x0, double inv)
{
  const double t = fmin(fmax(floor((v - x0) * inv), -1.0), (double)(n - 1));
  const int g = (int)t;
  auto above = [&](double a) { return STRICT ? a > v : a >= v; };
  const bool lo_ok = (g < 0) || !above(ax[g]);
  const bool hi_ok = (g + 1 >= n) || above(ax[g + 1]);
  if (lo_ok && hi_ok) return g + 1;
  int lo = 0, hi = n;
  while (lo < hi) { const int mid = (lo + hi) >> 1; if (above(ax[mid])) hi = mid; else lo = mid + 1; }
  return lo;
}

struct RectQuery { int j0, j1; int nw; int wa[3], wb[3]; };

__device__ __forceinline__ RectQuery d_rect_query(const FgRect &R, double lat_in_min, double lat_in_max, double lon_in_min, double lon_in_max)
{
  RectQuery q{};
  const double lon0 = R.hdr[0], inv_lon = R.hdr[1], lat0 = R.hdr[2], inv_lat = R.hdr[3];
  q.j0 = max(d_axis_first<true>(R.lat_ax, R.ny + 1, lat_in_min, lat0, inv_lat) - 1, 0);
  q.j1 = min(d_axis_first<false>(R.lat_ax, R.ny + 1, lat_in_max, lat0, inv_lat) - 1, R.ny - 1);
  q.nw = 0;
  if (lon_in_max - lon_in_min > G_PI) { q.nw = 1; q.wa[0] = 0; q.wb[0] = R.nx - 1; return q; }
  const double axl = R.lon_ax[0], axh = R.lon_ax[R.nx];
#pragma unroll
  for (int t = 2; t >= -2; t--) {
    const double T = t * G_TPI;
    const double lo = lon_in_min - RECT_EPS - T, hi = lon_in_max + RECT_EPS - T;
    if (!(axh > lo) || !(axl < hi)) continue;
    const int a = max(d_axis_first<true>(R.lon_ax, R.nx + 1, lo, lon0, inv_lon) - 1, 0);
    const int b = min(d_axis_first<false>(R.lon_ax, R.nx + 1, hi, lon0, inv_lon) - 1, R.nx - 1);
    if (a <= b && q.nw < 3) {
      if (q.nw == 0) { q.wa[0] = a; q.wb[0] = b; } else if (q.nw == 1) { q.wa[1] = a; q.wb[1] = b; } else { q.wa[2] = a; q.wb[2] = b; }
      q.nw++;
    }
  }
  return q;
}
__device__ __forceinline__ int d_rect_ncols(const RectQuery &q)
{
  int n = 0;
#pragma unroll
  for (int w = 0; w < 3; w++) if (w < q.nw) n += q.wb[w] - q.wa[w] + 1;
  return n;
}
__device__ __forceinline__ bool d_rect_heavy(const FgRect &R, double lat_in_min, double lat_in_max, double lon_in_min, double lon_in_max)
{
  const double nr = (lat_in_max - lat_in_min) * R.hdr[3] + 2.0;
  const double nc = (lon_in_max - lon_in_min > G_PI) ? (double)R.nx : (lon_in_max - lon_in_min) * R.hdr[1] + 2.0;
  return nr * nc > (double)RECT_HEAVY;
}
__device__ __forceinline__ int d_rect_col(const RectQuery &q, int k)
{
  int i = q.wa[0] + k;
  const int l0 = q.wb[0] - q.wa[0] + 1;
  if (q.nw > 1 && k >= l0) { i = q.wa[1] + (k - l0); const int l1 = q.wb[1] - q.wa[1] + 1; if (q.nw > 2 && k - l0 >= l1) i = q.wa[2] + (k - l0 - l1); }
  return i;
}
__device__ __forceinline__ bool d_rect_col_pass(const FgRect &R, int i, double lon_in_min, double lon_in_max, double lon_in_avg)
{
  double lon_out_min = R.col_min[i], lon_out_max = R.col_max[i];
  const double dx = R.col_avg[i] - lon_in_avg;
  if (dx < -G_PI)     { lon_out_min += G_TPI; lon_out_max += G_TPI; }
  else if (dx > G_PI) { lon_out_min -= G_TPI; lon_out_max -= G_TPI; }
  return !(lon_out_min >= lon_in_max || lon_out_max <= lon_in_min);
}

__device__ __forceinline__ double d_rect_area(const double *c, const double *r)
{
  const double s_lo = r[0], s_hi = r[4], s_mid = r[1], dat = r[2];
  const bool flat_m = r[3] != 0.0;
  double area = 0.0;
#pragma unroll
  for (int k = 0; k < 4; k++) {
    double dx = c[(k + 1) & 3] - c[k];
    if (dx > G_PI)  dx = dx - 2.0 * G_PI;
    if (dx < -G_PI) dx = dx + 2.0 * G_PI;
    if (fabs(dx + G_PI) < G_SMALL || fabs(dx - G_PI) < G_SMALL) { area += G_PI; continue; }
    if (k == 0) area -= dx * s_lo;
    else if (k == 2) area -= dx * s_hi;
    else if (flat_m) area -= dx * s_mid;
    else area -= dx * s_mid * dat;
  }
  if (area < 0) return -area * G_RADIUS * G_RADIUS;
  return area * G_RADIUS * G_RADIUS;
}

__device__ __forceinline__ int d_kth_set_bit(unsigned long long m, unsigned k)
{
  int pos = 0;
#pragma unroll
  for (int w = 32; w; w >>= 1) {
    const unsigned c = (unsigned)__popcll(m & ((1ull << w) - 1ull));
    if (k >= c) { k -= c; m >>= w; pos += w; }
  }
  return pos;
}

#define RECT_WL_WORDS 10
__device__ __forceinline__ bool d_rect_wave_candidates(const FgRect &R, const FgPairSpace &ps, bool active, int s, int nsrc, unsigned wave_no,
                                                       double lat_in_min, double lat_in_max, double lon_in_min, double lon_in_max,
                                                       double lon_in_avg, int *pair_beg, int *pair_cnt, int *big_list, int *big_cnt,
                                                       unsigned *wl )
{
  const int lane = threadIdx.x & 63;
  int cnt = 0, nr = 0, nwc = 0, nc = 0;
  unsigned long long cmask = 0ull;
  RectQuery q{};
  bool heavy = false;
  if (active) {
    heavy = d_rect_heavy(R, lat_in_min, lat_in_max, lon_in_min, lon_in_max);
    if (!heavy) {
      q = d_rect_query(R, lat_in_min, lat_in_max, lon_in_min, lon_in_max);
      nr = max(q.j1 - q.j0 + 1, 0);
      nwc = d_rect_ncols(q);
      if (nr > 0) {
        for (int k = 0; k < nwc; k++)
          if (d_rect_col_pass(R, d_rect_col(q, k), lon_in_min, lon_in_max, lon_in_avg)) { nc++; if (k < 64) cmask |= 1ull << k; }
      }
      cnt = (int)min((long)nr * nc, 0x3fffffffL);
    }
  }
  const unsigned incl = wave_incl_scan((unsigned)cnt, lane);
  const unsigned total = __shfl(incl, 63);
  const unsigned excl = incl - (unsigned)cnt;
  const int r = (int)((wave_no * 2654435761u >> 12) % (unsigned)ps.nreg);
  unsigned base = 0;
  if (lane == 0 && total) base = atomicAdd(&ps.fill[r * FG_FILL_STRIDE], total);
  base = __shfl(base, 0);
  int n_ok = 0;
  const unsigned first = base + excl;
  if (s < nsrc && !heavy) {
    const int loc0 = (int)min(first, (unsigned)ps.regcap);
    n_ok = min(cnt, ps.regcap - loc0);
    pair_beg[s] = r * ps.regcap + loc0;
    pair_cnt[s] = n_ok;
  }
  {
    const bool bigc = n_ok > CP_SMALL;
    const unsigned long long bm = __ballot(bigc);
    if (bm) {
      int qq = 0;
      if (lane == 0) qq = atomicAdd(big_cnt, __popcll(bm));
      qq = __shfl(qq, 0);
      if (bigc) big_list[qq + __popcll(bm & ((1ull << lane) - 1ull))] = s;
    }
  }
  const bool wide = nwc > 64;
  const int l0 = q.nw > 1 ? q.wb[0] - q.wa[0] + 1 : 64, l1 = q.nw > 2 ? q.wb[1] - q.wa[1] + 1 : 64;
  __syncthreads();
  wl[lane] = excl;
  wl[64 + lane] = wide ? 0u : (unsigned)nc;
  wl[2 * 64 + lane] = (unsigned)cmask; wl[3 * 64 + lane] = (unsigned)(cmask >> 32);
  wl[4 * 64 + lane] = (unsigned)q.j0;
  wl[5 * 64 + lane] = (unsigned)q.wa[0]; wl[6 * 64 + lane] = (unsigned)l0;
  wl[7 * 64 + lane] = (unsigned)(q.wa[1] - l0); wl[8 * 64 + lane] = (unsigned)(l0 + l1);
  wl[9 * 64 + lane] = (unsigned)(q.wa[2] - l0 - l1);
  __syncthreads();
  const unsigned lim = min(total, (unsigned)ps.regcap - min(base, (unsigned)ps.regcap));
  int *wsrc = ps.src + (size_t)r * ps.regcap + base, *wdst = ps.dst + (size_t)r * ps.regcap + base;
  const int s_first = s - lane;
  for (unsigned ob = 0; ob < lim; ob += 64) {
    const unsigned o = ob + lane;
    if (o >= lim || base + o >= (unsigned)ps.regcap) continue;
    int L = 0;
#pragma unroll
    for (int st = 32; st; st >>= 1) if (wl[L + st] <= o) L += st;
    const unsigned ncL = wl[64 + L];
    if (!ncL) continue;
    const unsigned t = o - wl[L], jr = t / ncL, kc = t - jr * ncL;
    const int k = d_kth_set_bit((unsigned long long)wl[2 * 64 + L] | ((unsigned long long)wl[3 * 64 + L] << 32), kc);
    const int i = k + (k < (int)wl[6 * 64 + L] ? (int)wl[5 * 64 + L] : k < (int)wl[8 * 64 + L] ? (int)wl[7 * 64 + L] : (int)wl[9 * 64 + L]);
    wsrc[o] = s_first + L;
    wdst[o] = ((int)wl[4 * 64 + L] + (int)jr) * R.nx + i;
  }
  if (wide && n_ok > 0) {
    int *psrc = ps.src + (size_t)r * ps.regcap + first, *pdst = ps.dst + (size_t)r * ps.regcap + first;
    int w = 0;
    for (int j = q.j0; j <= q.j1 && w < n_ok; j++)
      for (int k = 0; k < nwc && w < n_ok; k++) {
        const int i = d_rect_col(q, k);
        if (d_rect_col_pass(R, i, lon_in_min, lon_in_max, lon_in_avg)) { psrc[w] = s; pdst[w] = j * R.nx + i; w++; }
      }
  }
  return heavy;
}

__global__ __launch_bounds__(256, 4) void k_cell_struct2r(FgTileSet ts, const FgTile *tiles_in, FgTile *tiles_out, int ntiles, int nsrc, int ndst,
                                                        int nbS, FgCells S, double *area_out, FgRect R, const double *mask, int order, int *src_idx_f,
                                                        double *sums, unsigned *err, unsigned long long *band_keys, int cull,
                                                        int *heavy_list, int *heavy_cnt, FgPairSpace ps, int *pair_beg, int *pair_cnt,
                                                        int *big_list, int *big_cnt)
{
  __shared__ double vtile[256 * 17];
  __shared__ FgTile sh_tiles[FG_TILESET_MAX];
  static_assert(64 * RECT_WL_WORDS * sizeof(unsigned) <= 64 * 17 * sizeof(double), "a wave's share of vtile holds its candidate words");
  if (*R.bad) return;
  if (ts.n && (int)threadIdx.x < ts.n) sh_tiles[threadIdx.x] = ts.t[threadIdx.x];
  const bool isD = (int)blockIdx.x >= nbS;
  __shared__ unsigned long long sh_band[2];
  if (cull) {
    if (threadIdx.x == 0) { sh_band[0] = d_ord_key(R.lat_ax[R.ny]); sh_band[1] = ~d_ord_key(R.lat_ax[0]); }
    __syncthreads();
    band_keys = sh_band;
  }
  if (cull && !isD && band_keys[0]) {
    __syncthreads();
    const FgTile *tl0 = ts.n ? sh_tiles : tiles_in;
    const int s = blockIdx.x * 256 + threadIdx.x;
    bool keep = false;
    int idx_f = s;
    if (s < nsrc) {
      int t = 0;
      while (t + 1 < ntiles && s >= tl0[t + 1].cell_off) t++;
      const int loc = s - tl0[t].cell_off, i = loc % tl0[t].nx, j = loc / tl0[t].nx, nxp = tl0[t].nx + 1;
      if (order == 2) {
        int foff = 0;
        for (int m = 0; m < t; m++) foff += (tl0[m].nx + 2) * (tl0[m].ny + 2);
        idx_f = foff + (j + 1) * (tl0[t].nx + 2) + i + 1;
      }
      const int n0 = j * nxp + i;
      const double y0 = tl0[t].lat[n0], y1 = tl0[t].lat[n0 + 1], y2 = tl0[t].lat[n0 + nxp + 1], y3 = tl0[t].lat[n0 + nxp];
      const double lmin = fmin(fmin(y0, y1), fmin(y2, y3)), lmax = fmax(fmax(y0, y1), fmax(y2, y3));
      const double bmax = d_ord_val(band_keys[0]), bmin = d_ord_val(~band_keys[1]);
      keep = !((lmax <= bmin) || (lmin >= bmax)) || !(lmin == lmin);
    }
    if (!__syncthreads_or(keep)) {
      if (s < nsrc) {
        S.nv[s] = 0; S.area[s] = 0;
        pair_beg[s] = 0; pair_cnt[s] = 0;
        if (src_idx_f) src_idx_f[s] = idx_f;
        if (sums) { sums[s] = 0.0; sums[nsrc + s] = 0.0; sums[2 * (size_t)nsrc + s] = 0.0; }
      }
      if (ts.n && blockIdx.x == 0 && (int)threadIdx.x < ts.n) tiles_out[threadIdx.x] = sh_tiles[threadIdx.x];
      return;
    }
  }
  d_load_trig_table();
  const FgTile *tiles = ts.n ? sh_tiles : tiles_in;
  if (ts.n && blockIdx.x == 0 && (int)threadIdx.x < ts.n) tiles_out[threadIdx.x] = sh_tiles[threadIdx.x];
  if (!isD) {
    double box[5] = {0, 0, 0, 0, 0};
    int tl = 0;
    const int s0 = blockIdx.x * 256, s = s0 + threadIdx.x, lane = threadIdx.x & 63;
    const int nv = d_cell_record(tiles, ntiles, nsrc, S, err, s0, vtile, box, &tl, cull ? band_keys : nullptr);
    if (s < nsrc && sums) { sums[s] = 0.0; sums[nsrc + s] = 0.0; sums[2 * (size_t)nsrc + s] = 0.0; }
    if (s < nsrc && src_idx_f) {
      if (order != 2) src_idx_f[s] = s;
      else {
        int foff = 0;
        for (int t = 0; t < tl; t++) foff += (tiles[t].nx + 2) * (tiles[t].ny + 2);
        const int loc = s - tiles[tl].cell_off, i = loc % tiles[tl].nx, j = loc / tiles[tl].nx;
        src_idx_f[s] = foff + (j + 1) * (tiles[tl].nx + 2) + i + 1;
      }
    }
    const bool active = s < nsrc && nv > 0 && (!mask || mask[s] > 0.5);
    const bool heavy = d_rect_wave_candidates(R, ps, active, s, nsrc, (unsigned)(s >> 6), box[0], box[1], box[2], box[3], active ? S.lon_avg[s] : 0.0, pair_beg, pair_cnt,
                                              big_list, big_cnt, (unsigned *)(vtile + (threadIdx.x >> 6) * (64 * 17)));
    const unsigned long long m = __ballot(heavy);
    if (m) {
      int base = 0;
      if (lane == 0) base = atomicAdd(heavy_cnt, __popcll(m));
      base = __shfl(base, 0);
      if (heavy) heavy_list[base + __popcll(m & ((1ull << lane) - 1ull))] = s;
    }
  } else {
    const int d = ((int)blockIdx.x - nbS) * 256 + threadIdx.x;
    if (d < ndst) {
      const int j = d / R.nx, i = d - j * R.nx;
      area_out[d] = d_rect_area(R.col + (size_t)i * RECT_COLW, R.row + (size_t)j * 4);
    }
  }
}

__global__ __launch_bounds__(256) void k_polylist_records(FgPolyList P, FgCells S, int *src_idx_f, double *sums, FgRect R, int rect,
                                                           int *heavy_list, int *heavy_cnt, unsigned *err)
{
  if (rect && *R.bad) return;
  const int s = blockIdx.x * 256 + threadIdx.x, lane = threadIdx.x & 63;
  bool heavy = false;
  if (s < P.npoly) {
    const int n = P.n[s];
    double *v = S.verts + (size_t)s * 16;
    if (n < 3 || n > G_MAXV) {
      if (n > G_MAXV) atomicOr(err, G_ERRBIT_MAXV);
      S.nv[s] = 0; S.area[s] = 0; S.lat_min[s] = 0; S.lat_max[s] = 0; S.lon_min[s] = 0; S.lon_max[s] = 0; S.lon_avg[s] = 0;
      for (int k = 0; k < 16; k++) v[k] = 0.0;
    } else {
      double xmin = 0, xmax = 0, ymin = 0, ymax = 0;
      for (int k = 0; k < G_MAXV; k++) {
        const double x = (k < n) ? P.lon[(size_t)s * G_MAXV + k] : 0.0, y = (k < n) ? P.lat[(size_t)s * G_MAXV + k] : 0.0;
        v[k] = x; v[8 + k] = y;
        if (k == 0) { xmin = xmax = x; ymin = ymax = y; }
        else if (k < n) { xmin = fmin(xmin, x); xmax = fmax(xmax, x); ymin = fmin(ymin, y); ymax = fmax(ymax, y); }
      }
      if (!(ymin >= -G_HPI - 1.e-6) || !(ymax <= G_HPI + 1.e-6)) atomicOr(err, G_ERRBIT_BADLAT);
      S.nv[s] = n; S.area[s] = P.area[s]; S.lon_avg[s] = P.lon_avg[s];
      S.lat_min[s] = ymin; S.lat_max[s] = ymax; S.lon_min[s] = xmin; S.lon_max[s] = xmax;
      if (rect) heavy = d_rect_heavy(R, ymin, ymax, xmin, xmax);
    }
    if (src_idx_f) src_idx_f[s] = s;
    if (sums) { sums[s] = 0.0; sums[P.npoly + s] = 0.0; sums[2 * (size_t)P.npoly + s] = 0.0; }
  }
  if (rect) {
    const unsigned long long m = __ballot(heavy);
    if (m) {
      int base = 0;
      if (lane == 0) base = atomicAdd(heavy_cnt, __popcll(m));
      base = __shfl(base, 0);
      if (heavy) heavy_list[base + __popcll(m & ((1ull << lane) - 1ull))] = s;
    }
  }
}

__global__ __launch_bounds__(256) void k_rect_materialize(int ndst, FgRect R, FgCells D)
{
  const int d = blockIdx.x * 256 + threadIdx.x;
  if (d >= ndst) return;
  const int j = d / R.nx, i = d - j * R.nx;
  const double *c = R.col + (size_t)i * RECT_COLW;
  const double ya = R.lat_ax[j], yb = R.lat_ax[j + 1];
  D.lat_min[d] = ya; D.lat_max[d] = yb; D.lon_min[d] = c[4]; D.lon_max[d] = c[5]; D.lon_avg[d] = c[6]; D.nv[d] = 4;
  double *v = D.verts + (size_t)d * 16;
  for (int k = 0; k < 16; k++) v[k] = 0.0;
  v[0] = c[0]; v[1] = c[1]; v[2] = c[2]; v[3] = c[3];
  v[8] = ya; v[9] = ya; v[10] = yb; v[11] = yb;
}

__global__ __launch_bounds__(64) void k_candidates_rect(int nsrc, int H, FgCells S, const double *mask, FgRect R, FgPairSpace ps,
                                                         int *pair_beg, int *pair_cnt, const int *heavy_list, const int *heavy_cnt,
                                                         int *big_list, int *big_cnt)
{
  if (*R.bad) return;
  const int lane = threadIdx.x;
  if ((int)blockIdx.x < H) {
    const int nheavy = *heavy_cnt;
    for (int h = blockIdx.x; h < nheavy; h += H) {
      const int s = heavy_list[h];
      const double lon_in_min = S.lon_min[s], lon_in_max = S.lon_max[s], lon_in_avg = S.lon_avg[s];
      const RectQuery q = d_rect_query(R, S.lat_min[s], S.lat_max[s], lon_in_min, lon_in_max);
      const int nwc = d_rect_ncols(q), nr = q.j1 - q.j0 + 1;
      int nc = 0;
      for (int kb = 0; kb < nwc; kb += 64) {
        const int k = kb + lane;
        const bool pass = k < nwc && d_rect_col_pass(R, d_rect_col(q, k), lon_in_min, lon_in_max, lon_in_avg);
        nc += __popcll(__ballot(pass));
      }
      const long cnt_l = (long)nr * nc;
      const int cnt = (int)min(cnt_l, 0x7fffffffL);
      const int r = (int)(((unsigned)s * 2654435761u >> 12) % (unsigned)ps.nreg);
      unsigned base = 0;
      if (lane == 0 && cnt) base = atomicAdd(&ps.fill[r * FG_FILL_STRIDE], (unsigned)cnt);
      base = __shfl(base, 0);
      const int loc0 = (int)min(base, (unsigned)ps.regcap), n_ok = min(cnt, ps.regcap - loc0);
      const int wbase = r * ps.regcap + loc0;
      int cbase = 0;
      for (int kb = 0; kb < nwc && n_ok > 0; kb += 64) {
        const int k = kb + lane;
        int i = 0; bool pass = false;
        if (k < nwc) { i = d_rect_col(q, k); pass = d_rect_col_pass(R, i, lon_in_min, lon_in_max, lon_in_avg); }
        const unsigned long long m = __ballot(pass);
        const int at = cbase + __popcll(m & ((1ull << lane) - 1ull));
        if (pass)
          for (int jr = 0; jr < nr; jr++) {
            const long kk = (long)jr * nc + at;
            if (kk < n_ok) { ps.src[wbase + kk] = s; ps.dst[wbase + kk] = (q.j0 + jr) * R.nx + i; }
          }
        cbase += __popcll(m);
      }
      if (lane == 0) { pair_beg[s] = wbase; pair_cnt[s] = n_ok; if (n_ok > CP_SMALL) big_list[atomicAdd(big_cnt, 1)] = s; }
    }
    return;
  }
  __shared__ unsigned wl[64 * RECT_WL_WORDS];
  const int bR = (int)blockIdx.x - H;
  const int s = bR * 64 + lane;
  const bool active = s < nsrc && d_src_active(S, mask, s);
  double b[5] = {0, 0, 0, 0, 0};
  if (active) { b[0] = S.lat_min[s]; b[1] = S.lat_max[s]; b[2] = S.lon_min[s]; b[3] = S.lon_max[s]; b[4] = S.lon_avg[s]; }
  (void)d_rect_wave_candidates(R, ps, active, s, nsrc, (unsigned)bR, b[0], b[1], b[2], b[3], b[4], pair_beg, pair_cnt, big_list, big_cnt, wl);
}

struct ClipOut { double area, clon, clat; };

template <int ORDER, int S>
__device__ __forceinline__ void d_finish_pair(const double *px, const double *py, int n_out, double maskv,
                                              double area_in, double area_out, double lon_in_avg,
                                              ClipOut *o, unsigned long long *stats)
{
  double pa, clon = 0, clat = 0;
  if (ORDER == 2) d_poly_area_ctr<S>(px, py, n_out, lon_in_avg, &pa, &clon, &clat);
  else pa = d_poly_area<S>(px, py, n_out);
  double xarea = pa * maskv;
  double min_area = (area_in < area_out) ? area_in : area_out;
  double ratio = xarea / min_area;
  if (fabs(ratio - 1.e-6) < 1.e-15) atomicAdd(&stats[FG_STAT_BORDERLINE], 1ull);
  if (ratio > 1.e-6) { o->area = xarea; o->clon = clon; o->clat = clat; }
  else o->area = -2.0;
}

#ifndef CLIP_THREADS
#define CLIP_THREADS 256
#endif
#ifndef CLIP_SLOTS
#define CLIP_SLOTS 8
#endif
#ifndef CLIP_WAVES
#define CLIP_WAVES 4
#endif
#ifndef CLIP_PAD_LDS
#define CLIP_PAD_LDS 0
#endif

template <bool RECT, int T>
__device__ __forceinline__ int d_clip_quad_sh(double2 (*sh_poly)[T], const int tid, const int s, const int d,
                                              const FgCells &S, const FgCells &D, const FgRect &R, unsigned *err)
{
  constexpr int NV1 = RECT ? CLIP_SLOTS : 4;
  const double *sv = S.verts + (size_t)s * 16;
  double x1[NV1], y1[NV1], x2[4], y2[4];
  double lon_out_avg;
  int n1 = S.nv[s], n2 = RECT ? 4 : D.nv[d];
  double lon_in_avg = S.lon_avg[s];
#pragma unroll
  for (int k = 0; k < NV1; k++) { x1[k] = sv[k]; y1[k] = sv[8 + k]; }
  if (RECT) {
    const int j = d / R.nx, i = d - j * R.nx;
    const double *c = R.col + (size_t)i * RECT_COLW;
    double ya = R.lat_ax[j], yb = R.lat_ax[j + 1];
    x2[0] = c[0]; x2[1] = c[1]; x2[2] = c[2]; x2[3] = c[3]; lon_out_avg = c[6];
    asm volatile("" : "+v"(ya), "+v"(yb));
    y2[0] = ya; y2[1] = ya; y2[2] = yb; y2[3] = yb;
  } else {
    const double *dv = D.verts + (size_t)d * 16;
#pragma unroll
    for (int k = 0; k < 4; k++) { x2[k] = dv[k]; y2[k] = dv[8 + k]; }
    lon_out_avg = D.lon_avg[d];
#pragma unroll
    for (int k = 0; k < 4; k++) asm volatile("" : "+v"(y2[k]));
    asm volatile("" : "+v"(n2));
  }
#pragma unroll
  for (int k = 0; k < NV1; k++) asm volatile("" : "+v"(x1[k]), "+v"(y1[k]));
#pragma unroll
  for (int k = 0; k < 4; k++) asm volatile("" : "+v"(x2[k]));
  asm volatile("" : "+v"(n1), "+v"(lon_in_avg), "+v"(lon_out_avg));
  if (n1 > NV1 || n2 > 4) return -1;
  double shift = 0.0;
  {
    double dx = lon_out_avg - lon_in_avg;
    if (dx < -G_PI) shift = G_TPI; else if (dx > G_PI) shift = -G_TPI;
  }
  bool wrap = false;
#pragma unroll
  for (int k = 0; k < NV1; k++) {
    if (!(k < 4 || k < n1)) { x1[k] = 0.0; y1[k] = 0.0; }
    if (k < n1 && (x1[k] > G_TPI || x1[k] < 0.0)) wrap = true;
  }
#pragma unroll
  for (int k = 0; k < 4; k++) if (shift != 0.0) x2[k] += shift;
  if (wrap) {
#pragma unroll
    for (int k = 0; k < NV1; k++) x1[k] = d_pimod1(x1[k]);
#pragma unroll
    for (int k = 0; k < 4; k++) x2[k] = d_pimod1(x2[k]);
  }
#pragma unroll
  for (int k = 0; k < NV1; k++) if (k < 4 || k < n1) sh_poly[k][tid] = make_double2(x1[k], y1[k]);
  const long long b0x = __double_as_longlong(x2[0]), b1x = __double_as_longlong(x2[1]);
  const long long b2x = __double_as_longlong(x2[2]), b3x = __double_as_longlong(x2[3]);
  const long long b0y = __double_as_longlong(y2[0]), b1y = __double_as_longlong(y2[1]);
  const long long b2y = __double_as_longlong(y2[2]), b3y = __double_as_longlong(y2[3]);
  auto cut = [=](int e) -> double2 {
    const long long m0 = -(long long)(e == 0), m1 = -(long long)(e == 1), m2 = -(long long)(e == 2), m3 = -(long long)(e == 3);
    return make_double2(__longlong_as_double((b0x & m0) | (b1x & m1) | (b2x & m2) | (b3x & m3)),
                        __longlong_as_double((b0y & m0) | (b1y & m1) | (b2y & m2) | (b3y & m3)));
  };
  int n_cur = n1;
  bool overflow = false, parallel = false;
  double2 e0 = cut(n2 - 1);
#if FG_EXP == 2
  for (int e = 0; e < 0; e++) {
#else
#pragma unroll
  for (int e = 0; e < 4; e++) {
    if ((!RECT && e >= n2) || n_cur <= 0) break;
#endif
    double2 e1 = cut(e);
    const double x2_0 = e0.x, y2_0 = e0.y, x2_1 = e1.x, y2_1 = e1.y;
    double2 c[CLIP_SLOTS];
    unsigned inmask = 0u;
#pragma unroll
    for (int k = 0; k < CLIP_SLOTS; k++) c[k] = sh_poly[k][tid];
#pragma unroll
    for (int k = 0; k < CLIP_SLOTS; k++)
      if (k < n_cur) inmask |= (unsigned)d_inside_edge(x2_0, y2_0, x2_1, y2_1, c[k].x, c[k].y) << k;
    const unsigned full = (1u << n_cur) - 1u;
    const unsigned prevmask = ((inmask << 1) | (inmask >> (n_cur - 1))) & full;
    const unsigned tmask = inmask ^ prevmask;
    const int ncross = __popc(tmask);
    if (ncross > 2 || ncross + __popc(inmask) > CLIP_SLOTS) { overflow = true; break; }
    if (tmask) {
      const int ka = __ffs((int)tmask) - 1, kb = 31 - __clz((int)tmask);
      double2 I[2];
#pragma unroll
      for (int j = 0; j < 2; j++) {
        const int k = j ? kb : ka;
        const double2 p0 = sh_poly[k ? k - 1 : n_cur - 1][tid], p1 = sh_poly[k][tid];
        const double x1_0 = p0.x, y1_0 = p0.y, x1_1 = p1.x, y1_1 = p1.y;
        double dy1 = y1_1 - y1_0;
        double dy2 = y2_1 - y2_0;
        double dx1 = x1_1 - x1_0;
        double dx2 = x2_1 - x2_0;
        double ds1 = y1_0 * x1_1 - y1_1 * x1_0;
        double ds2 = y2_0 * x2_1 - y2_1 * x2_0;
        double determ = dy2 * dx1 - dy1 * dx2;
        if (fabs(determ) < 1.0e-30) parallel = true;
        I[j] = make_double2((dx2 * ds1 - dx1 * ds2) / determ, (dy2 * ds1 - dy1 * ds2) / determ);
      }
#pragma unroll
      for (int k = 0; k < CLIP_SLOTS; k++)
        if (k < n_cur && ((inmask >> k) & 1u))
          sh_poly[__popc(inmask & ((1u << k) - 1u)) + __popc(tmask & ((2u << k) - 1u))][tid] = c[k];
      sh_poly[__popc(inmask & ((1u << ka) - 1u))][tid] = I[0];
      sh_poly[__popc(inmask & ((1u << kb) - 1u)) + 1][tid] = I[1];
    }
    n_cur = ncross + __popc(inmask);
    e0 = e1;
  }
  if (overflow) return -1;
  if (parallel) atomicOr(err, G_ERRBIT_PARALLEL);
  return n_cur;
}
// ... 151 lines not shown
    for (int k = 0; k < n1; k++) {
      double xv = sv[k]; if (wrap) xv = d_pimod1(xv);
      sh_a[k][tid] = make_double2(xv, sv[8 + k]);
    }
#pragma unroll
    for (int k = 0; k < G_MAXV; k++)
      if (k < n2) {
        double xv = dvx[k]; if (shift != 0.0) xv += shift; if (wrap) xv = d_pimod1(xv);
        sh_cut[k][tid] = make_double2(xv, dvy[k]);
      }
    double2 (*cur)[GEN_THREADS] = sh_a;
    double2 (*nxt)[GEN_THREADS] = sh_b;
    int n_cur = n1;
    bool overflow = false, parallel = false;
    double2 e0 = sh_cut[n2 - 1][tid];
    for (int e = 0; e < n2 && n_cur > 0 && !overflow; e++) {
      double2 e1 = sh_cut[e][tid];
      const double x2_0 = e0.x, y2_0 = e0.y, x2_1 = e1.x, y2_1 = e1.y;
      double2 lastv = cur[n_cur - 1][tid];
      double x1_0 = lastv.x, y1_0 = lastv.y;
      int inside_last = d_inside_edge(x2_0, y2_0, x2_1, y2_1, x1_0, y1_0);
      int n_new = 0;
      for (int k = 0; k < n_cur; k++) {
        double2 cv = cur[k][tid];
        double x1_1 = cv.x, y1_1 = cv.y;
        int inside = d_inside_edge(x2_0, y2_0, x2_1, y2_1, x1_1, y1_1);
        if (inside != inside_last) {
          double dy1 = y1_1 - y1_0;
          double dy2 = y2_1 - y2_0;
          double dx1 = x1_1 - x1_0;
          double dx2 = x2_1 - x2_0;
          double ds1 = y1_0 * x1_1 - y1_1 * x1_0;
          double ds2 = y2_0 * x2_1 - y2_1 * x2_0;
          double determ = dy2 * dx1 - dy1 * dx2;
          if (fabs(determ) < 1.0e-30) parallel = true;
          if (n_new < GEN_CAP) nxt[n_new][tid] = make_double2((dx2 * ds1 - dx1 * ds2) / determ,
                                                              (dy2 * ds1 - dy1 * ds2) / determ);
          else overflow = true;
          n_new++;
        }
        if (inside) {
          if (n_new < GEN_CAP) nxt[n_new][tid] = make_double2(x1_1, y1_1);
          else overflow = true;
          n_new++;
        }
        x1_0 = x1_1; y1_0 = y1_1; inside_last = inside;
      }
      n_cur = n_new;
      double2 (*t)[GEN_THREADS] = cur; cur = nxt; nxt = t;
      e0 = e1;
    }
    if (overflow) { atomicOr(err, G_ERRBIT_OVERFLOW); pair_dst[p] = -1; continue; }
    if (parallel) atomicOr(err, G_ERRBIT_PARALLEL);
    ClipOut o; o.area = -1.0; o.clon = 0; o.clat = 0;
    if (n_cur > 0) {
      const double *px = (const double *)&cur[0][tid];
      d_finish_pair<ORDER, 2 * GEN_THREADS>(px, px + 1, n_cur, mask ? mask[s] : 1.0, S.area[s], D.area[d],
                                            lon_in_avg, &o, stats);
    }
    if (o.area >= 0) {
      tmp_area[p] = o.area;
      if (ORDER == 2) { tmp_clon[p] = o.clon; tmp_clat[p] = o.clat; }
      atomicAdd(&nacc[s], 1);
      if (row_cnt) tmp_rowpos[p] = atomicAdd(&row_cnt[d], 1);
    } else {
      pair_dst[p] = -1;
      if (o.area == -2.0) atomicAdd(&stats[FG_STAT_BELOW], 1ull);
    }
  }
}

#define CP_SPAN (256 + CP_SMALL)
static_assert(CP_SMALL % 64 == 0 && CP_SMALL <= 256, "the halo lanes of k_compact are whole waves of its 256-lane block");

struct CpPair { int s, d, beg, cnt, row; long x0; int na; double a, l, t; bool mine; };

__device__ __forceinline__ int d_row_slot(int *row_cnt, bool take, int d, int lane)
{
  const int key = take ? d : -1 - lane;
  const int prev = __shfl_up(key, 1, 64);
  const bool head = (lane == 0) || (key != prev);
  const unsigned long long hm = __ballot(head), am = __ballot(take);
  int slot = 0;
  if (!am) return 0;
  if (4 * __popcll(hm & am) > 3 * __popcll(am)) {
    if (take) slot = atomicAdd(&row_cnt[d], 1);
    return slot;
  }
  unsigned long long rem = am;
  for (int it = 0; rem && it < 8; it++) {
    const int lead = __ffsll((long long)rem) - 1;
    const int d0 = __shfl(d, lead);
    const unsigned long long grp = __ballot(take && d == d0) & rem;
    int base = 0;
    if (lane == lead) base = atomicAdd(&row_cnt[d0], __popcll(grp));
    base = __shfl(base, lead);
    if ((grp >> lane) & 1ull) slot = base + __popcll(grp & ((1ull << lane) - 1ull));
    rem &= ~grp;
  }
  if ((rem >> lane) & 1ull) slot = atomicAdd(&row_cnt[d], 1);
  return slot;
}

template <int ORDER, bool HALO>
__device__ __forceinline__ void d_cp_load(const FgPairSpace &ps, const FgCompactIo &io, int p0, int tid, unsigned live_end, CpPair &c, CpPair &h)
{
  constexpr int N = HALO ? 2 : 1;
  const int *const rowpos = io.tmp_rowpos ? io.tmp_rowpos : ps.dst;
  int p[N], pc[N], s[N], d[N], rp[N], beg[N], cnt[N], rb[N], x0[N], x1[N];
  bool ok[N];
  double a[N], l[N], t[N];
#pragma unroll
  for (int k = 0; k < N; k++) { p[k] = p0 + 256 * k + tid; ok[k] = (unsigned)p[k] < live_end; pc[k] = ok[k] ? p[k] : p0; }
#pragma unroll
  for (int k = 0; k < N; k++) {
    s[k] = ps.src[pc[k]]; d[k] = ps.dst[pc[k]]; rp[k] = rowpos[pc[k]];
    if (k == 0) { a[k] = io.tmp_area[pc[k]]; if (ORDER == 2) { l[k] = io.tmp_clon[pc[k]]; t[k] = io.tmp_clat[pc[k]]; } }
  }
#pragma unroll
  for (int k = 0; k < N; k++) {
    beg[k] = io.pair_beg[s[k]]; cnt[k] = io.pair_cnt[s[k]]; rb[k] = io.row_ptr[max(d[k], 0)];
    x0[k] = io.xoff[s[k]]; x1[k] = io.xoff[s[k] + 1];
  }
#pragma unroll
  for (int k = 0; k < N; k++) {
    const bool mine = ok[k] && cnt[k] <= CP_SMALL && beg[k] >= p0 && beg[k] < p0 + 256;
    if (k == 1) {
      a[k] = 0; l[k] = 0; t[k] = 0;
      if (mine && d[k] >= 0) { a[k] = io.tmp_area[p[k]]; if (ORDER == 2) { l[k] = io.tmp_clon[p[k]]; t[k] = io.tmp_clat[p[k]]; } }
    }
    CpPair &o = k ? h : c;
    o.s = ok[k] ? s[k] : 0; o.d = ok[k] ? d[k] : -1; o.beg = ok[k] ? beg[k] : 0; o.cnt = ok[k] ? cnt[k] : 0;
    o.mine = mine; o.x0 = mine ? x0[k] : 0; o.na = mine ? x1[k] - x0[k] : 0; o.row = (int)((unsigned)rb[k] + (unsigned)rp[k]);
    o.a = a[k]; o.l = (ORDER == 2) ? l[k] : 0.0; o.t = (ORDER == 2) ? t[k] : 0.0;
  }
}

template <int ORDER>
__device__ __forceinline__ long d_cp_place(const FgCompactIo &io, const CpPair &c, int p0, const int *sh_d, double (*sh_v)[CP_SPAN])
{
  if (!c.mine || c.d < 0 || c.x0 + c.na > io.xcap) return -1;
  int rank = 0;
  const int lb = c.beg - p0;
  for (int j = 0; j < c.cnt; j++) rank += ((unsigned)sh_d[lb + j] < (unsigned)c.d) ? 1 : 0;
  const long pos = c.x0 + rank;
  io.x_src[pos] = c.s; io.x_dst[pos] = c.d; io.x_area[pos] = c.a;
  if (ORDER == 2) { io.x_c1[pos] = c.l; io.x_c2[pos] = c.t; sh_v[0][lb + rank] = c.a; sh_v[1][lb + rank] = c.l; sh_v[2][lb + rank] = c.t; }
  if (io.tmp_rowpos) io.perm[c.row] = FgRowEnt{(int)pos, c.s};
  else return pos;
  return -1;
}

#define RANK_WORDS 1024
#define BIG_STAGE 512
#define BIG_BLOCKS 512
#define CP_LDS_DOUBLES (RANK_WORDS + RANK_WORDS / 2 + 3 * BIG_STAGE)

template <int ORDER>
__device__ __forceinline__ void d_compact_big(int nsrc, const FgPairSpace &ps, const FgCompactIo &io, double *lds)
{
  unsigned long long *bits = (unsigned long long *)lds;
  int *pref = (int *)(lds + RANK_WORDS);
  double (*sval)[BIG_STAGE] = (double (*)[BIG_STAGE])(lds + RANK_WORDS + RANK_WORDS / 2);
  __shared__ int smin, smax;
  if (blockIdx.x == 0 && threadIdx.x < 64) {
    unsigned long long f = 0; unsigned mx = 0;
    for (int r = threadIdx.x; r < ps.nreg; r += 64) { const unsigned v = ps.fill[r * FG_FILL_STRIDE]; f += v; mx = max(mx, v); }
#pragma unroll
    for (int o = 32; o; o >>= 1) { f += __shfl_xor(f, o); mx = max(mx, (unsigned)__shfl_xor((int)mx, o)); }
    if (threadIdx.x == 0) { io.dc->total[1] = f; io.dc->total[3] = mx; }
  }
  const int nb = *io.big_cnt;
  for (int h = blockIdx.x; h < nb; h += BIG_BLOCKS) {
    const int s = io.big_list[h];
    const int o = io.pair_beg[s], c = io.pair_cnt[s];
    const long x0 = io.xoff[s];
    const int na = io.xoff[s + 1] - (int)x0;
    if (threadIdx.x == 0) { smin = 0x7fffffff; smax = -1; }
    __syncthreads();
    int lmin = 0x7fffffff, lmax = -1;
    for (int k = threadIdx.x; k < c; k += 256) { const int d = ps.dst[o + k]; if (d >= 0) { lmin = min(lmin, d); lmax = max(lmax, d); } }
    if (lmax >= 0) { atomicMin(&smin, lmin); atomicMax(&smax, lmax); }
    __syncthreads();
    const int dmin = smin, dmax = smax;
    const long span = (long)dmax - dmin + 1;
    const bool bitmap = dmax >= 0 && span <= (long)RANK_WORDS * 64;
    if (bitmap) {
      const int nw = (int)((span + 63) >> 6);
      for (int w = threadIdx.x; w < nw; w += 256) bits[w] = 0ull;
      __syncthreads();
      for (int k = threadIdx.x; k < c; k += 256) {
        const int d = ps.dst[o + k];
        if (d >= 0) atomicOr(&bits[(d - dmin) >> 6], 1ull << ((d - dmin) & 63));
      }
      __syncthreads();
      const int per = (nw + 255) / 256, w0 = threadIdx.x * per, w1 = min(nw, w0 + per);
      int mine = 0;
      for (int w = w0; w < w1; w++) mine += __popcll(bits[w]);
      unsigned tot;
      const int before = (int)block_incl_scan((unsigned)mine, &tot) - mine;
      int run = before;
      for (int w = w0; w < w1; w++) { pref[w] = run; run += __popcll(bits[w]); }
      __syncthreads();
    }
    const bool ahead = na <= BIG_STAGE;
    const int *const rowpos = io.tmp_rowpos ? io.tmp_rowpos : ps.dst;
    double acc = 0;
    for (int c0 = 0; c0 < max(na, 1); c0 += BIG_STAGE) {
      for (int k = threadIdx.x; k < c; k += 256) {
        const int p = o + k;
        const int d = ps.dst[p];
        double a = 0, l = 0, t = 0;
        int row = 0;
        if (ahead) {
          a = io.tmp_area[p]; if (ORDER == 2) { l = io.tmp_clon[p]; t = io.tmp_clat[p]; }
          row = (int)((unsigned)rowpos[p] + (unsigned)io.row_ptr[max(d, 0)]);
        }
        if (d < 0) continue;
        int rank;
        if (bitmap) { const int w = (d - dmin) >> 6, b = (d - dmin) & 63; rank = pref[w] + __popcll(bits[w] & ((1ull << b) - 1ull)); }
        else { rank = 0; for (int j = 0; j < c; j++) rank += ((unsigned)ps.dst[o + j] < (unsigned)d) ? 1 : 0; }
        if (rank < c0 || rank >= c0 + BIG_STAGE) continue;
        const long pos = x0 + rank;
        if (pos >= io.xcap) continue;
        if (!ahead) {
          a = io.tmp_area[p]; if (ORDER == 2) { l = io.tmp_clon[p]; t = io.tmp_clat[p]; }
          if (io.tmp_rowpos) row = io.row_ptr[d] + io.tmp_rowpos[p];
        }
        io.x_src[pos] = s; io.x_dst[pos] = d; io.x_area[pos] = a;
        if (ORDER == 2) {
          io.x_c1[pos] = l; io.x_c2[pos] = t;
          sval[0][rank - c0] = a; sval[1][rank - c0] = l; sval[2][rank - c0] = t;
        }
        if (io.tmp_rowpos) io.perm[row] = FgRowEnt{(int)pos, s};
        else io.x_rowpos[pos] = atomicAdd(&io.row_cnt[d], 1);
      }
      __syncthreads();
      if (ORDER == 2 && threadIdx.x < 3 && x0 + na <= io.xcap) {
        const double *v = sval[threadIdx.x];
        const int n = min(BIG_STAGE, na - c0);
        int k = 0;
        for (; k + 8 <= n; k += 8) {
          double t[8];
#pragma unroll
          for (int u = 0; u < 8; u++) t[u] = v[k + u];
#pragma unroll
          for (int u = 0; u < 8; u++) acc += t[u];
        }
        for (; k < n; k++) acc += v[k];
      }
      __syncthreads();
    }
    if (ORDER == 2 && io.sums && threadIdx.x < 3) io.sums[(size_t)threadIdx.x * nsrc + s] = acc;
  }
}

template <int ORDER>
__global__ __launch_bounds__(256) void k_compact(int nsrc, FgPairSpace ps, FgCompactIo io)
{
  __shared__ double lds[CP_LDS_DOUBLES];
  if ((int)blockIdx.x < BIG_BLOCKS) { d_compact_big<ORDER>(nsrc, ps, io, lds); return; }
  int *sh_d = (int *)lds;
  double (*sh_v)[CP_SPAN] = (double (*)[CP_SPAN])(lds + CP_SPAN / 2 + 8);
  const int tid = threadIdx.x;
  const int p0 = ((int)blockIdx.x - BIG_BLOCKS) * 256;
  const unsigned r = (unsigned)p0 / (unsigned)ps.regcap;
  const unsigned rfill = ps.fill[r * FG_FILL_STRIDE];
  const unsigned live_end = r * (unsigned)ps.regcap + (rfill < (unsigned)ps.regcap ? rfill : (unsigned)ps.regcap);
  if ((unsigned)p0 >= live_end) return;
  CpPair c, h; h.mine = false; h.d = -1;
  if (tid < CP_SMALL) { d_cp_load<ORDER, true>(ps, io, p0, tid, live_end, c, h); sh_d[256 + tid] = h.d; }
  else d_cp_load<ORDER, false>(ps, io, p0, tid, live_end, c, h);
  sh_d[tid] = c.d;
  __syncthreads();
  const bool first = (unsigned)(p0 + tid) < live_end && p0 + tid == c.beg;
  {
    const long pos = d_cp_place<ORDER>(io, c, p0, sh_d, sh_v);
    if (!io.tmp_rowpos) { const int slot = d_row_slot(io.row_cnt, pos >= 0, c.d, tid & 63); if (pos >= 0) io.x_rowpos[pos] = slot; }
  }
  if (tid < CP_SMALL) {
    const long pos = d_cp_place<ORDER>(io, h, p0, sh_d, sh_v);
    if (!io.tmp_rowpos) { const int slot = d_row_slot(io.row_cnt, pos >= 0, h.d, tid & 63); if (pos >= 0) io.x_rowpos[pos] = slot; }
  }
  if (ORDER != 2 || !io.sums) return;
  __syncthreads();
  if (!first || !c.mine || c.x0 + c.na > io.xcap) return;
  double sa = 0, sl = 0, st = 0;
  const int lb = c.beg - p0;
  for (int k = 0; k < c.na; k++) { sa += sh_v[0][lb + k]; sl += sh_v[1][lb + k]; st += sh_v[2][lb + k]; }
  io.sums[c.s] = sa; io.sums[nsrc + c.s] = sl; io.sums[2 * (size_t)nsrc + c.s] = st;
}

__global__ __launch_bounds__(256) void k_centroids(int nsrc, FgCells S, const double *sums, FgSrcRec *cen)
{
  const int s = blockIdx.x * blockDim.x + threadIdx.x;
  double a = 0, ca = 1, cl = 0, ct = 0;
  int nv = 0;
  bool whole = false;
  if (s < nsrc && (a = sums[s]) > 0) {
    const double sl = sums[nsrc + s], st = sums[2 * (size_t)nsrc + s], sa = S.area[s];
    nv = S.nv[s];
    if (nv > 0) {
      ca = sa;
      if (fabs(a - ca) / ca < 1.e-3) {
        cl = sl / a;
        ct = st / a;
      } else whole = true;
    }
  }
  if (__syncthreads_or(whole)) {
    d_load_trig_table();
    if (whole) {
      double x[G_MAXV], y[G_MAXV];
      int n = nv;
      const double *vp = S.verts + (size_t)s * 16;
      for (int k = 0; k < G_MAXV; k++) { x[k] = vp[k]; y[k] = vp[8 + k]; }
      cl = d_poly_ctrlon<1>(x, y, n, S.lon_avg[s]) / ca;
      ct = d_poly_ctrlat<1>(x, y, n) / ca;
    }
  }
  if (s < nsrc) cen[s] = FgSrcRec{cl, ct};
}

__global__ __launch_bounds__(256) void k_distances(long nx, const int *x_src, const double *x_area, const FgSrcRec *cen, double *x_c1,
                                                    double *x_c2)
{
  long n = (long)blockIdx.x * blockDim.x + threadIdx.x;
  if (n >= nx) return;
  int s = x_src[n];
  double a = x_area[n];
  double di = x_c1[n] / a, dj = x_c2[n] / a;
  di -= cen[s].cen_lon; dj -= cen[s].cen_lat;
  x_c1[n] = di; x_c2[n] = dj;
}

static inline int nblk(long n, int t) { return (int)((n + t - 1) / t); }

void fgd_cell_struct(const FgTile *tiles_dev, int ntiles, int ncells, FgCells c, unsigned *err, hipStream_t st)
{
  if (ncells > 0) k_cell_struct<<<nblk(ncells, 256), 256, 0, st>>>(tiles_dev, ntiles, ncells, c, err);
}

void fgd_cell_struct2(const FgTileSet &ts, const FgTile *tiles_in, FgTile *tiles_out, int ntiles, int nsrc, int ndst, FgCells S, FgCells D,
                      FgBins b, int *slot_cnt, int order, int *src_idx_f, double *sums, unsigned *err, hipStream_t st,
                      unsigned long long *band_keys, int cull, double dst_tlon)
{
  const int nbS = nblk(nsrc, 256), nbD = nblk(ndst, 256);
  if (nbS + nbD > 0)
    k_cell_struct2<<<nbS + nbD, 256, 0, st>>>(ts, tiles_in, tiles_out, ntiles, nsrc, ndst, nbS, S, D, b, slot_cnt, order, src_idx_f, sums, err,
                                              band_keys, cull, dst_tlon);
}

void fgd_bin_count(int ncells, FgCells c, FgBins b, int *slot_cnt, hipStream_t st)
{
  if (ncells > 0) k_bin_count<<<nblk(ncells, 256), 256, 0, st>>>(ncells, c, b, slot_cnt);
}

void fgd_bin_fill(int ndst, FgCells D, FgBins b, int *slot_fill, const int *slot_start, FgBinEntry *entries, int cap,
                  int nsrc, FgCells S, const double *mask, int *heavy_list, int *heavy_cnt, hipStream_t st)
{
  const int nbD = nblk(ndst, 256), nbS = nblk(nsrc, 256);
  if (nbD + nbS > 0)
    k_bin_fill<<<nbD + nbS, 256, 0, st>>>(ndst, nbD, D, b, slot_fill, slot_start, entries, cap, nsrc, S, mask, heavy_list, heavy_cnt);
}

void fgd_candidates1(int nsrc, FgCells S, const double *mask, FgBins b, const int *slot_start, const FgBinEntry *entries, int ecap,
                     FgPairSpace ps, int *pair_beg, int *pair_cnt, const int *heavy_list, const int *heavy_cnt, int *big_list, int *big_cnt,
                     hipStream_t st)
{
  if (nsrc <= 0) return;
  const int nbR = nblk((long)nsrc * CAND_G, 64);
  const int H = min(8 * HEAVY_BLOCKS, max(64, nblk(nsrc, 8)));
  k_candidates1<<<nbR + H, 64, 0, st>>>(nsrc, H, S, mask, b, slot_start, entries, ecap, ps, pair_beg, pair_cnt, heavy_list, heavy_cnt, big_list, big_cnt);
}

void fgd_clip_quad(int order, FgPairSpace ps, FgCells S, const double *mask, FgCells D,
                   double *tmp_area, double *tmp_clon, double *tmp_clat, int *nacc, int *defer_list, int *defer_cnt,
                   unsigned long long *stats, unsigned *err, hipStream_t st, const FgRect *rect, int *row_cnt, int *tmp_rowpos)
{
  const long np = fgd_pairs_total(ps);
  if (np <= 0) return;
  const FgRect R = rect ? *rect : FgRect{};
  const int g = nblk(np, CLIP_THREADS);
#define FG_LAUNCH_QUAD(O, RC) k_clip_quad<O, RC><<<g, CLIP_THREADS, 0, st>>>(ps, S, mask, D, R, tmp_area, tmp_clon, tmp_clat, nacc, defer_list, defer_cnt, stats, err, row_cnt, tmp_rowpos)
  if (order == 2) { if (rect) FG_LAUNCH_QUAD(2, true); else FG_LAUNCH_QUAD(2, false); }
  else            { if (rect) FG_LAUNCH_QUAD(1, true); else FG_LAUNCH_QUAD(1, false); }
#undef FG_LAUNCH_QUAD
}

void fgd_clip_general(int order, FgPairSpace ps, FgCells S, const double *mask, FgCells D,
                      double *tmp_area, double *tmp_clon, double *tmp_clat, int *nacc, int *defer_list, int *defer_cnt,
                      unsigned long long *stats, unsigned *err, hipStream_t st, const FgRect *rect, int *row_cnt, int *tmp_rowpos)
{
  const long np = fgd_pairs_total(ps);
  if (np <= 0) return;
  int grid = nblk(np, GEN_THREADS); if (grid > 1024) grid = 1024;
  const FgRect R = rect ? *rect : FgRect{};
#define FG_LAUNCH_GEN(O, RC) k_clip_general<O, RC><<<grid, GEN_THREADS, 0, st>>>(defer_list, defer_cnt, ps.src, ps.dst, S, mask, D, R, tmp_area, tmp_clon, tmp_clat, nacc, stats, err, row_cnt, tmp_rowpos)
  if (order == 2) { if (rect) FG_LAUNCH_GEN(2, true); else FG_LAUNCH_GEN(2, false); }
  else            { if (rect) FG_LAUNCH_GEN(1, true); else FG_LAUNCH_GEN(1, false); }
#undef FG_LAUNCH_GEN
}

void fgd_rect_tables(const double *lon, const double *lat, int nx, int ny, double *hdr, double *lat_ax, double *lon_ax, double *col,
                     double *col_min, double *col_max, double *col_avg, double *row, unsigned *bad, unsigned *err, hipStream_t st, double dst_tlon)
{
  const long np = (long)(nx + 1) * (ny + 1);
  const int g = (int)std::min<long>(1024, std::max<long>((np + 255) / 256, (std::max(nx, ny) + 1 + 255) / 256));
  k_rect_tables<<<std::max(g, 1), 256, 0, st>>>(lon, lat, nx, ny, hdr, lat_ax, lon_ax, col, col_min, col_max, col_avg, row, bad, err, dst_tlon);
}
void fgd_cell_struct2r(const FgTileSet &ts, const FgTile *tiles_in, FgTile *tiles_out, int ntiles, int nsrc, int ndst, FgCells S, double *area_out,
                       FgRect R, const double *mask, int order, int *src_idx_f, double *sums, unsigned *err, hipStream_t st,
                       unsigned long long *band_keys, int cull, int *heavy_list, int *heavy_cnt, FgPairSpace ps, int *pair_beg, int *pair_cnt,
                       int *big_list, int *big_cnt)
{
  const int nbS = nblk(nsrc, 256), nbD = nblk(ndst, 256);
  if (nbS + nbD > 0)
    k_cell_struct2r<<<nbS + nbD, 256, 0, st>>>(ts, tiles_in, tiles_out, ntiles, nsrc, ndst, nbS, S, area_out, R, mask, order, src_idx_f, sums, err,
                                               band_keys, cull, heavy_list, heavy_cnt, ps, pair_beg, pair_cnt, big_list, big_cnt);
}
void fgd_polylist_records(FgPolyList P, FgCells S, int *src_idx_f, double *sums, const FgRect *rect, int *heavy_list, int *heavy_cnt,
                          unsigned *err, hipStream_t st)
{
  if (P.npoly > 0)
    k_polylist_records<<<nblk(P.npoly, 256), 256, 0, st>>>(P, S, src_idx_f, sums, rect ? *rect : FgRect{}, rect ? 1 : 0, heavy_list, heavy_cnt, err);
}
void fgd_rect_materialize(int ndst, FgRect R, FgCells D, hipStream_t st)
{
  if (ndst > 0) k_rect_materialize<<<nblk(ndst, 256), 256, 0, st>>>(ndst, R, D);
}
void fgd_candidates_rect(int nsrc, FgCells S, const double *mask, FgRect R, FgPairSpace ps, int *pair_beg, int *pair_cnt,
                         const int *heavy_list, const int *heavy_cnt, int *big_list, int *big_cnt, hipStream_t st, int listed_only)
{
  if (nsrc <= 0) return;
  const int nbR = listed_only ? 0 : nblk(nsrc, 64);
  const int H = min(HEAVY_BLOCKS, max(64, nblk(nsrc, 8)));
  k_candidates_rect<<<nbR + H, 64, 0, st>>>(nsrc, H, S, mask, R, ps, pair_beg, pair_cnt, heavy_list, heavy_cnt, big_list, big_cnt);
}

void fgd_compact(int order, int nsrc, FgPairSpace ps, const FgCompactIo &io, hipStream_t st)
{
  if (nsrc <= 0) return;
  const long np = fgd_pairs_total(ps);
  if (order == 2) k_compact<2><<<BIG_BLOCKS + nblk(np, 256), 256, 0, st>>>(nsrc, ps, io);
  else            k_compact<1><<<BIG_BLOCKS + nblk(np, 256), 256, 0, st>>>(nsrc, ps, io);
}

void fgd_centroids(int nsrc, FgCells S, const double *sums, FgSrcRec *cen, hipStream_t st)
{
  if (nsrc > 0) k_centroids<<<nblk(nsrc, 256), 256, 0, st>>>(nsrc, S, sums, cen);
}

void fgd_distances(long nx, const int *x_src, const double *x_area, const FgSrcRec *cen, double *x_c1, double *x_c2, hipStream_t st)
{
  if (nx > 0) k_distances<<<nblk(nx, 256), 256, 0, st>>>(nx, x_src, x_area, cen, x_c1, x_c2);
}

__global__ __launch_bounds__(256) void k_accumulate_cell_sums(int n, const int *cells, int nsrc, const int *xoff, const double *xa,
                                                               const double *c1, const double *c2, double *total)
{
  const int i = blockIdx.x * blockDim.x + threadIdx.x;
  if (i >= n) return;
  const int s = cells ? cells[i] : i;
  if (s < 0 || s >= nsrc) return;
  const int b = xoff[s], e = xoff[s + 1];
  if (b >= e) return;
  double a0 = total[s], a1 = total[(size_t)nsrc + s], a2 = total[2 * (size_t)nsrc + s];
  for (int q = b; q < e; q++) { a0 += xa[q]; a1 += c1[q]; a2 += c2[q]; }
  total[s] = a0; total[(size_t)nsrc + s] = a1; total[2 * (size_t)nsrc + s] = a2;
}
void fgd_accumulate_cell_sums(int n, const int *cells, int nsrc, const int *xoff, const double *xa, const double *c1, const double *c2,
                              double *total, hipStream_t st)
{
  if (n > 0) k_accumulate_cell_sums<<<(n + 255) / 256, 256, 0, st>>>(n, cells, nsrc, xoff, xa, c1, c2, total);
}
```

Baseline: 5.530 billion exchange-cells/s.

## Specialize cell records to quads and defer rare cells to candidate pass

The rect cell-struct kernel now uses a quad-only record path with a smaller LDS tile (9 doubles per thread instead of 17), which raises its launch bound from 4 to 7 waves. Cells whose quick longitude fix fails are put on a rare list and finished, with their candidates, by dedicated blocks in the candidates kernel. Separately, k_compact's LDS staging is resized dynamically to fit eight blocks per CU. This cuts LDS and register pressure on the common path, at the cost of more code complexity and an extra pass for rare cells.

```diff
diff --git a/fre-nctools_amd/conserve_interp.py b/fre-nctools_amd/conserve_interp.py
--- a/fre-nctools_amd/conserve_interp.py
+++ b/fre-nctools_amd/conserve_interp.py
@@ -217,9 +217,9 @@
         check(lib().fg_plan_accumulate_cell_sums(*args))
 
     def stats(self):
-        s = (C.c_long * 10)()
-        check(lib().fg_plan_stats(self._h, s, 10))
-        names = ["pairs", "nonempty", "nxgrid", "borderline", "bins", "bin_entries", "deferred", "heavy", "below", "exact_mode"]
+        s = (C.c_long * 11)()
+        check(lib().fg_plan_stats(self._h, s, 11))
+        names = ["pairs", "nonempty", "nxgrid", "borderline", "bins", "bin_entries", "deferred", "heavy", "below", "exact_mode", "rare"]
         return dict(zip(names, [int(v) for v in s]))
 
     PHASES = ["cell_struct", "bins", "candidates", "clip_quad", "clip_general", "compact", "rows",
diff --git a/fre-nctools_amd/csrc/plan.hip b/fre-nctools_amd/csrc/plan.hip
--- a/fre-nctools_amd/csrc/plan.hip
+++ b/fre-nctools_amd/csrc/plan.hip
@@ -617,6 +617,7 @@
   char *zero_blk = blk.get<char>(zbytes);
   int *bin_start = blk.get<int>(nslots + 1);
   int *heavy_list = blk.get<int>(nsrc + 1);
+  int *rare_list = blk.get<int>(rect ? nsrc + 1 : 1);
   int *big_list = blk.get<int>(nsrc + 1);
   int *pair_beg = blk.get<int>(nsrc + 1), *pair_cnt = blk.get<int>(nsrc + 1);
   FgBinEntry *bin_entries = blk.get<FgBinEntry>(nentries ? nentries : 1);
@@ -674,7 +675,7 @@
     if (pl->polys.npoly) fgd_polylist_records(pl->polys, pl->S, pl->src_idx_f, pl->sums, &R, heavy_list, &dc->heavy_cnt, dc->err, st);
     fgd_cell_struct2r(ts, pl->tiles_dev, pl->tiles_dev, pl->ntiles, pl->polys.npoly ? 0 : nsrc, ndst, pl->S, pl->D.area, R, pl->mask_dev, order,
                       pl->src_idx_f, pl->sums, dc->err, st, dc->band_keys, (opt.cull && !pl->polys.npoly) ? 2 : 0, heavy_list, &dc->heavy_cnt,
-                      ps, pair_beg, pair_cnt, big_list, &dc->big_cnt);
+                      rare_list, &dc->rare_cnt, ps, pair_beg, pair_cnt, big_list, &dc->big_cnt);
   } else if (opt.cull && !boxm && !pl->polys.npoly) {
     fgd_band_keys(in.lat_out, (long)(pl->nx_out + 1) * (pl->ny_out + 1), dc->band_keys, st);
     fgd_cell_struct2(ts, pl->tiles_dev, pl->tiles_dev, pl->ntiles, nsrc, ndst, pl->S, pl->D, bins, bin_cnt, order, pl->src_idx_f, pl->sums, dc->err, st, dc->band_keys, 2, dst_tlon);
@@ -699,7 +700,8 @@
   pt.begin(PH_CANDIDATES);
   if (rect)
     fgd_candidates_rect(nsrc, pl->S, pl->mask_dev, pl->rect_tab, ps, pair_beg, pair_cnt, heavy_list, &dc->heavy_cnt, big_list, &dc->big_cnt, st,
-                        pl->polys.npoly ? 0 : 1);
+                        pl->polys.npoly ? 0 : 1,
+                        rare_list, &dc->rare_cnt, dc->err);
   else
     fgd_candidates1(nsrc, pl->S, pl->mask_dev, bins, bin_start, bin_entries, ecap, ps, pair_beg, pair_cnt, heavy_list, &dc->heavy_cnt, big_list,
                     &dc->big_cnt, st);
@@ -804,6 +806,7 @@
   pl->stats[FG_STAT_BIN_ENTRIES] = (long)hc->total[0];
   pl->stats[FG_STAT_DEFERRED] = hc->defer_cnt + hc->gc_list2_cnt;
   pl->stats[FG_STAT_HEAVY] = hc->heavy_cnt;
+  pl->stats[FG_STAT_RARE] = hc->rare_cnt;
   pl->stats[FG_STAT_BELOW] = (long)hc->stats[FG_STAT_BELOW];
 
   pl->rect_tab.bad = nullptr;
diff --git a/fre-nctools_amd/csrc/xgrid_device.h b/fre-nctools_amd/csrc/xgrid_device.h
--- a/fre-nctools_amd/csrc/xgrid_device.h
+++ b/fre-nctools_amd/csrc/xgrid_device.h
@@ -45,7 +45,8 @@
   FG_STAT_HEAVY = 7,
   FG_STAT_BELOW = 8,
   FG_STAT_EXACT = 9,
-  FG_NSTATS = 10
+  FG_STAT_RARE = 10,
+  FG_NSTATS = 11
 };
 
 #define FG_REG_ALIGN 512
@@ -97,6 +98,7 @@
   unsigned rect_bad;
   int defer_cnt, big_cnt;
   int gc_list2_cnt;
+  int rare_cnt;
   unsigned long long stats[FG_NSTATS];
 };
 #define G_ERRBIT_LOOKBACK 128u
@@ -136,14 +138,15 @@
                      double dst_tlon = 3.14159265358979323846);
 void fgd_cell_struct2r(const FgTileSet &ts, const FgTile *tiles_in, FgTile *tiles_out, int ntiles, int nsrc, int ndst, FgCells S, double *area_out,
                        FgRect R, const double *mask, int order, int *src_idx_f, double *sums, unsigned *err, hipStream_t st,
-                       unsigned long long *band_keys, int cull, int *heavy_list, int *heavy_cnt, FgPairSpace ps, int *pair_beg, int *pair_cnt,
-                       int *big_list, int *big_cnt);
+                       unsigned long long *band_keys, int cull, int *heavy_list, int *heavy_cnt, int *rare_list, int *rare_cnt, FgPairSpace ps,
+                       int *pair_beg, int *pair_cnt, int *big_list, int *big_cnt);
 void fgd_rect_materialize(int ndst, FgRect R, FgCells D, hipStream_t st);
 struct FgPolyList { const int *n; const double *lon, *lat; const double *lon_avg, *area; int npoly; };
 void fgd_polylist_records(FgPolyList P, FgCells S, int *src_idx_f, double *sums, const FgRect *rect, int *heavy_list, int *heavy_cnt,
                           unsigned *err, hipStream_t st);
 void fgd_candidates_rect(int nsrc, FgCells S, const double *mask, FgRect R, FgPairSpace ps, int *pair_beg, int *pair_cnt,
-                         const int *heavy_list, const int *heavy_cnt, int *big_list, int *big_cnt, hipStream_t st, int listed_only);
+                         const int *heavy_list, const int *heavy_cnt, int *big_list, int *big_cnt, hipStream_t st, int listed_only,
+                         const int *rare_list = nullptr, const int *rare_cnt = nullptr, unsigned *err = nullptr);
 void fgd_clip_general(int order, FgPairSpace ps, FgCells S, const double *mask, FgCells D,
               double *tmp_area, double *tmp_clon, double *tmp_clat, int *nacc, int *defer_list, int *defer_cnt,
               unsigned long long *stats, unsigned *err, hipStream_t st, const FgRect *rect = nullptr, int *row_cnt = nullptr,
diff --git a/fre-nctools_amd/csrc/xgrid_kernels.hip b/fre-nctools_amd/csrc/xgrid_kernels.hip
--- a/fre-nctools_amd/csrc/xgrid_kernels.hip
+++ b/fre-nctools_amd/csrc/xgrid_kernels.hip
@@ -191,15 +191,18 @@
 }
 
 
+template <bool QUADS_ONLY = false>
 __device__ __forceinline__ int d_cell_record(const FgTile *tiles, int ntiles, int ncells, const FgCells &c, unsigned *err, int s0,
                                              double *vtile, double *box , int *tile_of,
-                                             const unsigned long long *cull = nullptr, double tlon = G_PI)
-{
+                                             const unsigned long long *cull = nullptr, double tlon = G_PI, bool *rare = nullptr)
+{
+  constexpr int VS = QUADS_ONLY ? 9 : 17, NLIVE = QUADS_ONLY ? 8 : 16, CAP = QUADS_ONLY ? 4 : G_FIXCAP;
   const int s = s0 + threadIdx.x;
-  double *row = vtile + threadIdx.x * 17;
-#pragma unroll
-  for (int k = 0; k < 16; k++) row[k] = 0.0;
+  double *row = vtile + threadIdx.x * VS;
+#pragma unroll
+  for (int k = 0; k < NLIVE; k++) row[k] = 0.0;
   int nvert = 0;
+  bool listed = false;
   if (s < ncells) {
     int t = 0;
     while (t + 1 < ntiles && s >= tiles[t + 1].cell_off) t++;
@@ -209,7 +212,7 @@
     int i = loc % T.nx, j = loc / T.nx;
     int nxp = T.nx + 1;
     int n0 = j * nxp + i, n1 = n0 + 1, n3 = n0 + nxp, n2 = n3 + 1;
-    double x[G_FIXCAP], y[G_FIXCAP];
+    double x[CAP], y[CAP];
     x[0] = T.lon[n0]; y[0] = T.lat[n0];
     x[1] = T.lon[n1]; y[1] = T.lat[n1];
     x[2] = T.lon[n2]; y[2] = T.lat[n2];
@@ -226,11 +229,32 @@
       out_of_band = (lmax <= bmin) || (lmin >= bmax);
     }
     int n = out_of_band ? 0 : d_fix_lon_quad_fast(x, y, tlon);
-    if (n < 0) n = d_fix_lon(x, y, 4, tlon);
+    if constexpr (!QUADS_ONLY) {
+      if (n < 0) n = d_fix_lon(x, y, 4, tlon);
+    }
     if (out_of_band) { c.nv[s] = 0; c.area[s] = 0; }
+    else if (QUADS_ONLY && n < 0) {
+      listed = true;
+#pragma unroll
+      for (int k = 0; k < 4; k++) { row[k] = x[k]; row[4 + k] = y[k]; }
+    }
     else if (n < 0 || n > G_MAXV) {
       atomicOr(err, G_ERRBIT_MAXV);
       c.nv[s] = 0; c.lon_min[s] = 0; c.lon_max[s] = 0; c.lon_avg[s] = 0; c.area[s] = 0;
+    } else if constexpr (QUADS_ONLY) {
+      double xmin = x[0], xmax = x[0], xs = 0;
+#pragma unroll
+      for (int k = 1; k < 4; k++) { if (x[k] < xmin) xmin = x[k]; if (x[k] > xmax) xmax = x[k]; }
+#pragma unroll
+      for (int k = 0; k < 4; k++) xs += x[k];
+      xs /= 4;
+      c.lon_min[s] = xmin; c.lon_max[s] = xmax; c.lon_avg[s] = xs;
+      box[2] = xmin; box[3] = xmax; box[4] = xs;
+      c.nv[s] = 4;
+      nvert = 4;
+#pragma unroll
+      for (int k = 0; k < 4; k++) { row[k] = x[k]; row[4 + k] = y[k]; }
+      c.area[s] = d_poly_area<1>(x, y, 4);
     } else {
       double xmin = x[0], xmax = x[0], xs = 0;
       for (int k = 1; k < n; k++) { if (x[k] < xmin) xmin = x[k]; if (x[k] > xmax) xmax = x[k]; }
@@ -247,15 +271,56 @@
       c.area[s] = d_poly_area<1>(x, y, n);
     }
   }
-  if (!__syncthreads_or(nvert != 0) && cull) return 0;
+  if (QUADS_ONLY) *rare = listed;
+  if (!__syncthreads_or(nvert != 0 || listed) && cull) return 0;
   const long cnt = (long)min(256, ncells - s0) * 16;
   double *out = c.verts + (size_t)s0 * 16;
 #pragma unroll
   for (int q = 0; q < 16; q++) {
     const long e = (long)q * 256 + threadIdx.x;
-    if (e < cnt) out[e] = vtile[(e >> 4) * 17 + (e & 15)];
+    if constexpr (QUADS_ONLY) {
+      const int k = (int)e & 15;
+      if (e < cnt) out[e] = (k & 4) ? 0.0 : vtile[(e >> 4) * VS + ((k >> 3) << 2) + (k & 3)];
+    } else if (e < cnt) out[e] = vtile[(e >> 4) * VS + (e & 15)];
   }
   return nvert;
+}
+
+__device__ __forceinline__ int d_finish_rare_cell(const FgCells &c, unsigned *err, int s, int lane, double *box)
+{
+  double *v = c.verts + (size_t)s * 16;
+  double x[G_FIXCAP], y[G_FIXCAP];
+#pragma unroll
+  for (int k = 0; k < 4; k++) { x[k] = v[k]; y[k] = v[8 + k]; }
+  double lmin = y[0], lmax = y[0];
+#pragma unroll
+  for (int k = 1; k < 4; k++) { if (y[k] < lmin) lmin = y[k]; if (y[k] > lmax) lmax = y[k]; }
+  box[0] = lmin; box[1] = lmax;
+  const int n = d_fix_lon(x, y, 4, G_PI);
+  if (n < 0 || n > G_MAXV) {
+    if (lane == 0) {
+      atomicOr(err, G_ERRBIT_MAXV);
+      c.nv[s] = 0; c.lon_min[s] = 0; c.lon_max[s] = 0; c.lon_avg[s] = 0; c.area[s] = 0;
+      for (int k = 0; k < 16; k++) v[k] = 0.0;
+    }
+    return 0;
+  }
+  double xmin = x[0], xmax = x[0], xs = 0;
+  for (int k = 1; k < n; k++) { if (x[k] < xmin) xmin = x[k]; if (x[k] > xmax) xmax = x[k]; }
+  for (int k = 0; k < n; k++) xs += x[k];
+  xs /= n;
+  box[2] = xmin; box[3] = xmax; box[4] = xs;
+  const double area = d_poly_area<1>(x, y, n);
+  if (lane == 0) {
+    c.lon_min[s] = xmin; c.lon_max[s] = xmax; c.lon_avg[s] = xs;
+    c.nv[s] = n;
+    for (int k = 0; k < G_MAXV; k++) {
+      v[k] = (k < n) ? x[k] : 0.0;
+      v[8 + k] = (k < n) ? y[k] : 0.0;
+    }
+    c.area[s] = area;
+  }
+  return n;
 }
 
 __global__ __launch_bounds__(256) void k_cell_struct(const FgTile *tiles, int ntiles, int ncells, FgCells c, unsigned *err)
@@ -864,6 +929,7 @@
 }
 
 #define RECT_WL_WORDS 10
+template <bool ONE = false>
 __device__ __forceinline__ bool d_rect_wave_candidates(const FgRect &R, const FgPairSpace &ps, bool active, int s, int nsrc, unsigned wave_no,
                                                        double lat_in_min, double lat_in_max, double lon_in_min, double lon_in_max,
                                                        double lon_in_avg, int *pair_beg, int *pair_cnt, int *big_list, int *big_cnt,
@@ -896,7 +962,7 @@
   base = __shfl(base, 0);
   int n_ok = 0;
   const unsigned first = base + excl;
-  if (s < nsrc && !heavy) {
+  if (s < nsrc && !heavy && (!ONE || lane == 0)) {
     const int loc0 = (int)min(first, (unsigned)ps.regcap);
     n_ok = min(cnt, ps.regcap - loc0);
     pair_beg[s] = r * ps.regcap + loc0;
@@ -925,7 +991,7 @@
   __syncthreads();
   const unsigned lim = min(total, (unsigned)ps.regcap - min(base, (unsigned)ps.regcap));
   int *wsrc = ps.src + (size_t)r * ps.regcap + base, *wdst = ps.dst + (size_t)r * ps.regcap + base;
-  const int s_first = s - lane;
+  const int s_first = ONE ? s : s - lane;
   for (unsigned ob = 0; ob < lim; ob += 64) {
     const unsigned o = ob + lane;
     if (o >= lim || base + o >= (unsigned)ps.regcap) continue;
@@ -952,15 +1018,16 @@
   return heavy;
 }
 
-__global__ __launch_bounds__(256, 4) void k_cell_struct2r(FgTileSet ts, const FgTile *tiles_in, FgTile *tiles_out, int ntiles, int nsrc, int ndst,
+#define RECORD_WAVES 7
+__global__ __launch_bounds__(256, RECORD_WAVES) void k_cell_struct2r(FgTileSet ts, const FgTile *tiles_in, FgTile *tiles_out, int ntiles, int nsrc, int ndst,
                                                         int nbS, FgCells S, double *area_out, FgRect R, const double *mask, int order, int *src_idx_f,
                                                         double *sums, unsigned *err, unsigned long long *band_keys, int cull,
-                                                        int *heavy_list, int *heavy_cnt, FgPairSpace ps, int *pair_beg, int *pair_cnt,
-                                                        int *big_list, int *big_cnt)
-{
-  __shared__ double vtile[256 * 17];
+                                                        int *heavy_list, int *heavy_cnt, int *rare_list, int *rare_cnt, FgPairSpace ps,
+                                                        int *pair_beg, int *pair_cnt, int *big_list, int *big_cnt)
+{
+  __shared__ double vtile[256 * 9];
   __shared__ FgTile sh_tiles[FG_TILESET_MAX];
-  static_assert(64 * RECT_WL_WORDS * sizeof(unsigned) <= 64 * 17 * sizeof(double), "a wave's share of vtile holds its candidate words");
+  static_assert(64 * RECT_WL_WORDS * sizeof(unsigned) <= 64 * 9 * sizeof(double), "a wave's share of vtile holds its candidate words");
   if (*R.bad) return;
   if (ts.n && (int)threadIdx.x < ts.n) sh_tiles[threadIdx.x] = ts.t[threadIdx.x];
   const bool isD = (int)blockIdx.x >= nbS;
@@ -1009,7 +1076,17 @@
     double box[5] = {0, 0, 0, 0, 0};
     int tl = 0;
     const int s0 = blockIdx.x * 256, s = s0 + threadIdx.x, lane = threadIdx.x & 63;
-    const int nv = d_cell_record(tiles, ntiles, nsrc, S, err, s0, vtile, box, &tl, cull ? band_keys : nullptr);
+    bool rare = false;
+    const int nv = d_cell_record<true>(tiles, ntiles, nsrc, S, err, s0, vtile, box, &tl, cull ? band_keys : nullptr, G_PI, &rare);
+    {
+      const unsigned long long m = __ballot(rare);
+      if (m) {
+        int base = 0;
+        if (lane == 0) base = atomicAdd(rare_cnt, __popcll(m));
+        base = __shfl(base, 0);
+        if (rare) rare_list[base + __popcll(m & ((1ull << lane) - 1ull))] = s;
+      }
+    }
     if (s < nsrc && sums) { sums[s] = 0.0; sums[nsrc + s] = 0.0; sums[2 * (size_t)nsrc + s] = 0.0; }
     if (s < nsrc && src_idx_f) {
       if (order != 2) src_idx_f[s] = s;
@@ -1021,8 +1098,8 @@
       }
     }
     const bool active = s < nsrc && nv > 0 && (!mask || mask[s] > 0.5);
-    const bool heavy = d_rect_wave_candidates(R, ps, active, s, nsrc, (unsigned)(s >> 6), box[0], box[1], box[2], box[3], active ? S.lon_avg[s] : 0.0, pair_beg, pair_cnt,
-                                              big_list, big_cnt, (unsigned *)(vtile + (threadIdx.x >> 6) * (64 * 17)));
+    const bool heavy = d_rect_wave_candidates(R, ps, active, s, nsrc, (unsigned)(s >> 6), box[0], box[1], box[2], box[3], box[4], pair_beg, pair_cnt,
+                                              big_list, big_cnt, (unsigned *)(vtile + (threadIdx.x >> 6) * (64 * 9)));
     const unsigned long long m = __ballot(heavy);
     if (m) {
       int base = 0;
@@ -1093,58 +1170,82 @@
   v[8] = ya; v[9] = ya; v[10] = yb; v[11] = yb;
 }
 
+__device__ __forceinline__ void d_rect_cell_candidates(const FgRect &R, const FgPairSpace &ps, int s, int lane, double lat_in_min, double lat_in_max,
+                                                       double lon_in_min, double lon_in_max, double lon_in_avg, int *pair_beg, int *pair_cnt,
+                                                       int *big_list, int *big_cnt)
+{
+  const RectQuery q = d_rect_query(R, lat_in_min, lat_in_max, lon_in_min, lon_in_max);
+  const int nwc = d_rect_ncols(q), nr = q.j1 - q.j0 + 1;
+  int nc = 0;
+  for (int kb = 0; kb < nwc; kb += 64) {
+    const int k = kb + lane;
+    const bool pass = k < nwc && d_rect_col_pass(R, d_rect_col(q, k), lon_in_min, lon_in_max, lon_in_avg);
+    nc += __popcll(__ballot(pass));
+  }
+  const long cnt_l = (long)nr * nc;
+  const int cnt = (int)min(cnt_l, 0x7fffffffL);
+  const int r = (int)(((unsigned)s * 2654435761u >> 12) % (unsigned)ps.nreg);
+  unsigned base = 0;
+  if (lane == 0 && cnt) base = atomicAdd(&ps.fill[r * FG_FILL_STRIDE], (unsigned)cnt);
+  base = __shfl(base, 0);
+  const int loc0 = (int)min(base, (unsigned)ps.regcap), n_ok = min(cnt, ps.regcap - loc0);
+  const int wbase = r * ps.regcap + loc0;
+  int cbase = 0;
+  for (int kb = 0; kb < nwc && n_ok > 0; kb += 64) {
+    const int k = kb + lane;
+    int i = 0; bool pass = false;
+    if (k < nwc) { i = d_rect_col(q, k); pass = d_rect_col_pass(R, i, lon_in_min, lon_in_max, lon_in_avg); }
+    const unsigned long long m = __ballot(pass);
+    const int at = cbase + __popcll(m & ((1ull << lane) - 1ull));
+    if (pass)
+      for (int jr = 0; jr < nr; jr++) {
+        const long kk = (long)jr * nc + at;
+        if (kk < n_ok) { ps.src[wbase + kk] = s; ps.dst[wbase + kk] = (q.j0 + jr) * R.nx + i; }
+      }
+    cbase += __popcll(m);
+  }
+  if (lane == 0) { pair_beg[s] = wbase; pair_cnt[s] = n_ok; if (n_ok > CP_SMALL) big_list[atomicAdd(big_cnt, 1)] = s; }
+}
+
+#define RARE_BLOCKS 64
+template <bool FINISH>
 __global__ __launch_bounds__(64) void k_candidates_rect(int nsrc, int H, FgCells S, const double *mask, FgRect R, FgPairSpace ps,
                                                          int *pair_beg, int *pair_cnt, const int *heavy_list, const int *heavy_cnt,
-                                                         int *big_list, int *big_cnt)
-{
-  if (*R.bad) return;
+                                                         int *big_list, int *big_cnt, const int *rare_list, const int *rare_cnt, unsigned *err)
+{
   const int lane = threadIdx.x;
-  if ((int)blockIdx.x < H) {
+  __shared__ unsigned wl[64 * RECT_WL_WORDS];
+  if (FINISH && (int)blockIdx.x < RARE_BLOCKS) d_load_trig_table();
+  const unsigned bad = *R.bad;
+  const int nrare = FINISH ? *rare_cnt : 0;
+  if (bad) return;
+  const int hb = FINISH ? (int)blockIdx.x - RARE_BLOCKS : (int)blockIdx.x;
+  if (hb >= 0 && hb < H) {
     const int nheavy = *heavy_cnt;
-    for (int h = blockIdx.x; h < nheavy; h += H) {
+    for (int h = hb; h < nheavy; h += H) {
       const int s = heavy_list[h];
-      const double lon_in_min = S.lon_min[s], lon_in_max = S.lon_max[s], lon_in_avg = S.lon_avg[s];
-      const RectQuery q = d_rect_query(R, S.lat_min[s], S.lat_max[s], lon_in_min, lon_in_max);
-      const int nwc = d_rect_ncols(q), nr = q.j1 - q.j0 + 1;
-      int nc = 0;
-      for (int kb = 0; kb < nwc; kb += 64) {
-        const int k = kb + lane;
-        const bool pass = k < nwc && d_rect_col_pass(R, d_rect_col(q, k), lon_in_min, lon_in_max, lon_in_avg);
-        nc += __popcll(__ballot(pass));
-      }
-      const long cnt_l = (long)nr * nc;
-      const int cnt = (int)min(cnt_l, 0x7fffffffL);
-      const int r = (int)(((unsigned)s * 2654435761u >> 12) % (unsigned)ps.nreg);
-      unsigned base = 0;
-      if (lane == 0 && cnt) base = atomicAdd(&ps.fill[r * FG_FILL_STRIDE], (unsigned)cnt);
-      base = __shfl(base, 0);
-      const int loc0 = (int)min(base, (unsigned)ps.regcap), n_ok = min(cnt, ps.regcap - loc0);
-      const int wbase = r * ps.regcap + loc0;
-      int cbase = 0;
-      for (int kb = 0; kb < nwc && n_ok > 0; kb += 64) {
-        const int k = kb + lane;
-        int i = 0; bool pass = false;
-        if (k < nwc) { i = d_rect_col(q, k); pass = d_rect_col_pass(R, i, lon_in_min, lon_in_max, lon_in_avg); }
-        const unsigned long long m = __ballot(pass);
-        const int at = cbase + __popcll(m & ((1ull << lane) - 1ull));
-        if (pass)
-          for (int jr = 0; jr < nr; jr++) {
-            const long kk = (long)jr * nc + at;
-            if (kk < n_ok) { ps.src[wbase + kk] = s; ps.dst[wbase + kk] = (q.j0 + jr) * R.nx + i; }
-          }
-        cbase += __popcll(m);
-      }
-      if (lane == 0) { pair_beg[s] = wbase; pair_cnt[s] = n_ok; if (n_ok > CP_SMALL) big_list[atomicAdd(big_cnt, 1)] = s; }
+      d_rect_cell_candidates(R, ps, s, lane, S.lat_min[s], S.lat_max[s], S.lon_min[s], S.lon_max[s], S.lon_avg[s], pair_beg, pair_cnt, big_list, big_cnt);
     }
     return;
   }
-  __shared__ unsigned wl[64 * RECT_WL_WORDS];
-  const int bR = (int)blockIdx.x - H;
-  const int s = bR * 64 + lane;
-  const bool active = s < nsrc && d_src_active(S, mask, s);
-  double b[5] = {0, 0, 0, 0, 0};
-  if (active) { b[0] = S.lat_min[s]; b[1] = S.lat_max[s]; b[2] = S.lon_min[s]; b[3] = S.lon_max[s]; b[4] = S.lon_avg[s]; }
-  (void)d_rect_wave_candidates(R, ps, active, s, nsrc, (unsigned)bR, b[0], b[1], b[2], b[3], b[4], pair_beg, pair_cnt, big_list, big_cnt, wl);
+  if constexpr (FINISH) {
+    for (int h = blockIdx.x; h < nrare; h += RARE_BLOCKS) {
+      const int s = rare_list[h];
+      const double mk = mask ? mask[s] : 1.0;
+      double b[5] = {0, 0, 0, 0, 0};
+      const int nv = d_finish_rare_cell(S, err, s, lane, b);
+      if (!(nv > 0 && mk > 0.5)) continue;
+      if (d_rect_heavy(R, b[0], b[1], b[2], b[3])) d_rect_cell_candidates(R, ps, s, lane, b[0], b[1], b[2], b[3], b[4], pair_beg, pair_cnt, big_list, big_cnt);
+      else (void)d_rect_wave_candidates<true>(R, ps, lane == 0, s, nsrc, (unsigned)(s >> 6), b[0], b[1], b[2], b[3], b[4], pair_beg, pair_cnt, big_list, big_cnt, wl);
+    }
+  } else {
+    const int bR = (int)blockIdx.x - H;
+    const int s = bR * 64 + lane;
+    const bool active = s < nsrc && d_src_active(S, mask, s);
+    double b[5] = {0, 0, 0, 0, 0};
+    if (active) { b[0] = S.lat_min[s]; b[1] = S.lat_max[s]; b[2] = S.lon_min[s]; b[3] = S.lon_max[s]; b[4] = S.lon_avg[s]; }
+    (void)d_rect_wave_candidates(R, ps, active, s, nsrc, (unsigned)bR, b[0], b[1], b[2], b[3], b[4], pair_beg, pair_cnt, big_list, big_cnt, wl);
+  }
 }
 
 struct ClipOut { double area, clon, clat; };
@@ -1602,16 +1703,17 @@
 }
 
 #define RANK_WORDS 1024
-#define BIG_STAGE 512
 #define BIG_BLOCKS 512
-#define CP_LDS_DOUBLES (RANK_WORDS + RANK_WORDS / 2 + 3 * BIG_STAGE)
+#define CP_LDS_DOUBLES 2552
+static_assert(CP_LDS_DOUBLES >= CP_SPAN / 2 + 8 + 3 * CP_SPAN, "the lane-per-pair role's sh_d and sh_v fit the block's LDS");
+static_assert(CP_LDS_DOUBLES >= RANK_WORDS + RANK_WORDS / 2 + 3 * 8, "a bitmap of full size leaves room for a stage");
+static_assert(8 * (CP_LDS_DOUBLES * 8 + 64) <= 160 * 1024, "eight blocks of k_compact per CU");
+__device__ __forceinline__ int d_big_stage(int nw) { const int w8 = (nw + 7) & ~7; return ((CP_LDS_DOUBLES - w8 - w8 / 2) / 3) & ~7; }
 
 template <int ORDER>
 __device__ __forceinline__ void d_compact_big(int nsrc, const FgPairSpace &ps, const FgCompactIo &io, double *lds)
 {
   unsigned long long *bits = (unsigned long long *)lds;
-  int *pref = (int *)(lds + RANK_WORDS);
-  double (*sval)[BIG_STAGE] = (double (*)[BIG_STAGE])(lds + RANK_WORDS + RANK_WORDS / 2);
   __shared__ int smin, smax;
   if (blockIdx.x == 0 && threadIdx.x < 64) {
     unsigned long long f = 0; unsigned mx = 0;
@@ -1635,8 +1737,11 @@
     const int dmin = smin, dmax = smax;
     const long span = (long)dmax - dmin + 1;
     const bool bitmap = dmax >= 0 && span <= (long)RANK_WORDS * 64;
+    const int nw = bitmap ? (int)((span + 63) >> 6) : 0, w8 = (nw + 7) & ~7;
+    int *pref = (int *)(lds + w8);
+    const int stage = d_big_stage(nw);
+    double *sval = lds + w8 + w8 / 2;
     if (bitmap) {
-      const int nw = (int)((span + 63) >> 6);
       for (int w = threadIdx.x; w < nw; w += 256) bits[w] = 0ull;
       __syncthreads();
       for (int k = threadIdx.x; k < c; k += 256) {
@@ -1653,10 +1758,10 @@
       for (int w = w0; w < w1; w++) { pref[w] = run; run += __popcll(bits[w]); }
       __syncthreads();
     }
-    const bool ahead = na <= BIG_STAGE;
+    const bool ahead = na <= stage;
     const int *const rowpos = io.tmp_rowpos ? io.tmp_rowpos : ps.dst;
     double acc = 0;
-    for (int c0 = 0; c0 < max(na, 1); c0 += BIG_STAGE) {
+    for (int c0 = 0; c0 < max(na, 1); c0 += stage) {
       for (int k = threadIdx.x; k < c; k += 256) {
         const int p = o + k;
         const int d = ps.dst[p];
@@ -1670,7 +1775,7 @@
         int rank;
         if (bitmap) { const int w = (d - dmin) >> 6, b = (d - dmin) & 63; rank = pref[w] + __popcll(bits[w] & ((1ull << b) - 1ull)); }
         else { rank = 0; for (int j = 0; j < c; j++) rank += ((unsigned)ps.dst[o + j] < (unsigned)d) ? 1 : 0; }
-        if (rank < c0 || rank >= c0 + BIG_STAGE) continue;
+        if (rank < c0 || rank >= c0 + stage) continue;
         const long pos = x0 + rank;
         if (pos >= io.xcap) continue;
         if (!ahead) {
@@ -1680,15 +1785,15 @@
         io.x_src[pos] = s; io.x_dst[pos] = d; io.x_area[pos] = a;
         if (ORDER == 2) {
           io.x_c1[pos] = l; io.x_c2[pos] = t;
-          sval[0][rank - c0] = a; sval[1][rank - c0] = l; sval[2][rank - c0] = t;
+          sval[rank - c0] = a; sval[stage + rank - c0] = l; sval[2 * stage + rank - c0] = t;
         }
         if (io.tmp_rowpos) io.perm[row] = FgRowEnt{(int)pos, s};
         else io.x_rowpos[pos] = atomicAdd(&io.row_cnt[d], 1);
       }
       __syncthreads();
       if (ORDER == 2 && threadIdx.x < 3 && x0 + na <= io.xcap) {
-        const double *v = sval[threadIdx.x];
-        const int n = min(BIG_STAGE, na - c0);
+        const double *v = sval + threadIdx.x * stage;
+        const int n = min(stage, na - c0);
         int k = 0;
         for (; k + 8 <= n; k += 8) {
           double t[8];
@@ -1706,7 +1811,7 @@
 }
 
 template <int ORDER>
-__global__ __launch_bounds__(256) void k_compact(int nsrc, FgPairSpace ps, FgCompactIo io)
+__global__ __launch_bounds__(256, 8) void k_compact(int nsrc, FgPairSpace ps, FgCompactIo io)
 {
   __shared__ double lds[CP_LDS_DOUBLES];
   if ((int)blockIdx.x < BIG_BLOCKS) { d_compact_big<ORDER>(nsrc, ps, io, lds); return; }
@@ -1861,13 +1966,13 @@
 }
 void fgd_cell_struct2r(const FgTileSet &ts, const FgTile *tiles_in, FgTile *tiles_out, int ntiles, int nsrc, int ndst, FgCells S, double *area_out,
                        FgRect R, const double *mask, int order, int *src_idx_f, double *sums, unsigned *err, hipStream_t st,
-                       unsigned long long *band_keys, int cull, int *heavy_list, int *heavy_cnt, FgPairSpace ps, int *pair_beg, int *pair_cnt,
-                       int *big_list, int *big_cnt)
+                       unsigned long long *band_keys, int cull, int *heavy_list, int *heavy_cnt, int *rare_list, int *rare_cnt, FgPairSpace ps,
+                       int *pair_beg, int *pair_cnt, int *big_list, int *big_cnt)
 {
   const int nbS = nblk(nsrc, 256), nbD = nblk(ndst, 256);
   if (nbS + nbD > 0)
     k_cell_struct2r<<<nbS + nbD, 256, 0, st>>>(ts, tiles_in, tiles_out, ntiles, nsrc, ndst, nbS, S, area_out, R, mask, order, src_idx_f, sums, err,
-                                               band_keys, cull, heavy_list, heavy_cnt, ps, pair_beg, pair_cnt, big_list, big_cnt);
+                                               band_keys, cull, heavy_list, heavy_cnt, rare_list, rare_cnt, ps, pair_beg, pair_cnt, big_list, big_cnt);
 }
 void fgd_polylist_records(FgPolyList P, FgCells S, int *src_idx_f, double *sums, const FgRect *rect, int *heavy_list, int *heavy_cnt,
                           unsigned *err, hipStream_t st)
@@ -1880,12 +1985,17 @@
   if (ndst > 0) k_rect_materialize<<<nblk(ndst, 256), 256, 0, st>>>(ndst, R, D);
 }
 void fgd_candidates_rect(int nsrc, FgCells S, const double *mask, FgRect R, FgPairSpace ps, int *pair_beg, int *pair_cnt,
-                         const int *heavy_list, const int *heavy_cnt, int *big_list, int *big_cnt, hipStream_t st, int listed_only)
+                         const int *heavy_list, const int *heavy_cnt, int *big_list, int *big_cnt, hipStream_t st, int listed_only,
+                         const int *rare_list, const int *rare_cnt, unsigned *err)
 {
   if (nsrc <= 0) return;
   const int nbR = listed_only ? 0 : nblk(nsrc, 64);
   const int H = min(HEAVY_BLOCKS, max(64, nblk(nsrc, 8)));
-  k_candidates_rect<<<nbR + H, 64, 0, st>>>(nsrc, H, S, mask, R, ps, pair_beg, pair_cnt, heavy_list, heavy_cnt, big_list, big_cnt);
+  const int Hf = max(H - RARE_BLOCKS, RARE_BLOCKS);
+  if (listed_only) k_candidates_rect<true><<<Hf + RARE_BLOCKS, 64, 0, st>>>(nsrc, Hf, S, mask, R, ps, pair_beg, pair_cnt, heavy_list, heavy_cnt, big_list, big_cnt,
+                                                          rare_list, rare_cnt, err);
+  else k_candidates_rect<false><<<nbR + H, 64, 0, st>>>(nsrc, H, S, mask, R, ps, pair_beg, pair_cnt, heavy_list, heavy_cnt, big_list, big_cnt,
+                                                       nullptr, nullptr, nullptr);
 }
 
 void fgd_compact(int order, int nsrc, FgPairSpace ps, const FgCompactIo &io, hipStream_t st)
```

Result: faster. 5.639 billion exchange-cells/s, median of 6 (+2.0%).
